# smpurkis/PyTorch-Face-Detection-from-Scratch

Measured on AMD Instinct MI355X. Metric: train imgs/sec (PoolResnet 480^2, bs=256 per GPU), higher is better.
Workload: dtype f32 (3x3 convs: bf16x3 split MFMA, fp32 accumulate)

## Files before the change

### include/fdet.h

```cpp
#ifndef FDET_H
#define FDET_H

#include <stddef.h>
#include <stdint.h>

#ifdef __cplusplus
extern "C" {
#endif

#define FDET_VERSION 100
#define FDET_OK 0
#define FDET_EINVAL (-1)
#define FDET_ELAUNCH (-2)
#define FDET_EWORKSPACE (-3)

int fdet_version(void);
const char* fdet_last_error(void);


int fdet_encode_targets(const float* boxes, const int32_t* box_offset, int B, int S,
                        float img_w, float img_h, float* out, void* stream);

int fdet_yolo_loss_fwd_bwd(const float* pred, const float* gt, int B, int S,
                           float* loss_per_image, float* loss_sum, float* grad_pred,
                           float grad_scale, void* stream);

int fdet_decode(const float* maps, int B, int S, float prob_threshold, float img_w, float img_h,
                float* scores, float* boxes, int32_t* counts, void* stream);

int fdet_nms(const float* boxes, const float* scores, const int32_t* counts, int B, int Kmax,
             double iou_threshold, int32_t* keep, int32_t* keep_counts, void* stream);

int fdet_reduce_bounding_boxes(const float* maps, int B, int S, float prob_threshold,
                               double iou_threshold, float img_w, float img_h,
                               float* out, int32_t* out_counts, void* stream);

int fdet_step_metrics(const float* gt, const int32_t* gt_counts, const float* pred,
                      const int32_t* pred_counts, int B, int Kmax, float* per_image,
                      float* totals, void* stream);

int fdet_u8_to_f32_norm(const uint8_t* in, float* out, size_t n, void* stream);


int fdet_adam_step(float* param, const float* grad, float* exp_avg, float* exp_avg_sq, size_t n,
                   int step, double lr, double beta1, double beta2, double eps, float grad_scale,
                   void* stream);

int fdet_ssd_num_priors(const int* h_patch_sizes, int nscales);
int fdet_ssd_encode_targets(const float* boxes, const int32_t* box_offsets, int B, const int* h_patch_sizes,
                            int nscales, float img_w, float img_h, float* out, void* stream);
size_t fdet_ssd_loss_ws_bytes(int B);
int fdet_ssd_loss_fwd_bwd(const float* pred, const float* target, int B, int P, int neg_pos_ratio, float* loss,
                          float* grad, uint8_t* mask, void* ws, size_t ws_bytes, void* stream);
int fdet_ssd_loss_parts(const float* pred, const float* target, int B, int P, int neg_pos_ratio, float* grad, uint8_t* mask,
                        double* sums, void* ws, size_t ws_bytes, void* stream);
int fdet_ssd_loss_finish(const double* sums, float* loss, float* grad, size_t n_grad, void* ws, size_t ws_bytes, void* stream);
int fdet_ssd_reduce_bounding_boxes(const float* x, int B, const int* h_patch_sizes, int nscales, int with_priors,
                                   float prob_threshold, double iou_threshold, float img_w, float img_h,
                                   float* out, int32_t* out_counts, void* stream);
int fdet_ssd_reduce_bounding_boxes_priors(const float* x, int B, const int* h_patch_sizes, int nscales, int with_priors,
                                          const float* priors, float prob_threshold, double iou_threshold, float img_w,
                                          float img_h, float* out, int32_t* out_counts, void* stream);

int fdet_ssd_head_pack_fwd(const float* z, int N, int CP, int ps, int prior_start, int P, float* y, void* stream);
int fdet_ssd_head_pack_bwd(const float* dy, const float* y, int N, int CP, int ps, int prior_start, int P, float* dz,
                           void* stream);

int fdet_resize_bilinear_u8_norm(const uint8_t* src, float* dst, int N, int C, int Hs, int Ws,
                                 int Hd, int Wd, void* stream);
int fdet_resize_bilinear_f32_norm(const float* src, float* dst, int N, int C, int Hs, int Ws,
                                  int Hd, int Wd, float divisor, void* stream);


int fdet_pack_conv3x3_weights(const float* w, int Cout, int Cin, float* wpk_fwd, float* wpk_bwd,
                              void* stream);

int fdet_conv3x3_fwd(const float* x, const float* wpk, const float* bias, float* y_full,
                     const float* skip, const float* drop_scale, float* y_out,
                     int N, int Cin, int Cout, int H, int W, int pool, float slope, void* stream);

int fdet_conv3x3_dgrad(const float* dz, const float* wpk, const float* act, const float* add,
                       float* dx, int N, int Cin, int Cout, int H, int W, float slope, void* stream);

int fdet_pack_conv3x3_weights_bf16x3(const float* w, int Cout, int Cin, void* wpk_fwd, void* wpk_bwd,
                                     void* stream);
int fdet_pack_conv3x3_weights_bf16x3_batched(const float* const* h_w, int L, int Cout, int Cin,
                                             void* const* h_wpk_fwd, void* const* h_wpk_bwd, void* stream);
int fdet_conv3x3_fwd_bf16x3(const float* x, const void* wpk, const float* bias, float* y_full,
                            const float* skip, const float* drop_scale, float* y_out,
                            int N, int Cin, int Cout, int H, int W, int pool, float slope, void* stream);
int fdet_conv3x3_dgrad_bf16x3(const float* dz, const void* wpk, const float* act, const float* add,
                              float* dx, int N, int Cin, int Cout, int H, int W, float slope, void* stream);

size_t fdet_conv3x3_wgrad_ws_bytes(int N, int Cin, int Cout, int H, int W);
int fdet_conv3x3_wgrad(const float* x, const float* dz, float* dW, float* db, void* ws,
                       size_t ws_bytes, int N, int Cin, int Cout, int H, int W, void* stream);

size_t fdet_conv3x3_wgrad_bf16x3_ws_bytes(int N, int Cin, int Cout, int H, int W);
int fdet_conv3x3_wgrad_bf16x3(const float* x, const float* dz, float* dW, float* db, void* ws,
                              size_t ws_bytes, int N, int Cin, int Cout, int H, int W, void* stream);

size_t fdet_conv3x3_wgrad_bf16x3_batched_ws_bytes(int L, int N, int Cin, int Cout, int H, int W);
int fdet_conv3x3_wgrad_bf16x3_plan(int N, int Cin, int Cout, int H, int W, int L, int* out, int n);
int fdet_conv3x3_wgrad_bf16x3_batched(const float* const* h_x, const float* const* h_dz, float* const* h_dW,
                                      float* const* h_db, int L, void* ws, size_t ws_bytes,
                                      int N, int Cin, int Cout, int H, int W, void* stream);

int fdet_block_chain_supported(int F, int H, int W);
int fdet_block_chain_ok(int N, int F, int H, int W, int ps);
int fdet_block_chain_fwd_bf16x3(const float* x, const void* const* h_wpk1, const float* const* h_b1,
                                const void* const* h_wpk2, const float* const* h_b2,
                                const float* const* h_scale, float* const* h_a, float* const* h_c,
                                float* const* h_out, int nblocks, int N, int F, int H, int W, float slope,
                                void* stream);
int fdet_block_chain_bwd_bf16x3(const float* dout, const void* const* h_wpk1b, const void* const* h_wpk2b,
                                const float* const* h_scale, const float* const* h_a, const float* const* h_c,
                                float* const* h_dz1, float* const* h_dz2, float* dx, int nblocks, int N, int F,
                                int H, int W, float slope, void* stream);

int fdet_block_chain_fwd_ps(const void* x, int x_is_ps, const void* const* h_wpk1, const float* const* h_b1,
                            const void* const* h_wpk2, const float* const* h_b2, const float* const* h_scale,
                            void* const* h_a_ps, void* const* h_c_ps, void* const* h_out_ps, float* out_last,
                            int nblocks, int N, int F, int H, int W, float slope, void* stream);
int fdet_block_chain_bwd_ps(const float* dout, const void* const* h_wpk1b, const void* const* h_wpk2b,
                            const float* const* h_scale, const void* const* h_a_ps, const void* const* h_c_ps,
                            void* const* h_dz1_ps, void* const* h_dz2_ps, float* dx, int nblocks, int N, int F,
                            int H, int W, float slope, void* stream);

int fdet_block_tail_fwd(const float* c, const float* x, const float* drop_scale, float* out,
                        int N, int F, int H, int W, int pool, void* stream);

int fdet_conv3x3_pool_fusion_ok(int N, int Cin, int Cout, int H, int W);
int fdet_conv3x3_x3_last_route(int* out, int n);
int fdet_conv3x3_ps_ok(int N, int Cin, int Cout, int H, int W, int pooled);
int fdet_conv3x3_fwd_pool_bf16x3(const float* x, const void* wpk, const float* bias, const float* skip,
                                 const float* drop_scale, float* out_pooled, unsigned char* route, int N, int Cin,
                                 int Cout, int H, int W, float slope, void* stream);
int fdet_conv3x3_dgrad_unpool_bf16x3(const float* dz, const void* wpk, const float* dout_pooled,
                                     const unsigned char* route, float* dx, int N, int Cin, int Cout, int H, int W,
                                     float slope, void* stream);
int fdet_pool_route_bwd(const float* dout_pooled, const unsigned char* route, const float* drop_scale, float* dz2,
                        int N, int F, int H, int W, float slope, void* stream);

size_t fdet_ps_bytes(int N, int C, int H, int W);
size_t fdet_ps_image0_offset(int N, int C, int H, int W);
int fdet_ps_from_f32(const float* x, void* ps, int N, int C, int H, int W, void* stream);
int fdet_ps_to_f32(const void* ps, float* x, int N, int C, int H, int W, void* stream);
int fdet_ps_strips(int W);
int fdet_ps_halo_exchange(void* ps, int N, int C, int H, int W, int zero_only, int hi_only, void* stream);
int fdet_conv3x3_ps_fwd(const void* x_ps, const void* wpk, const float* bias, void* y_ps, int N, int Cin, int Cout,
                        int H, int W, float slope, void* stream);
int fdet_conv3x3_ps_dgrad_act(const void* dz_ps, const void* wpk, const void* act_ps, void* dx_ps, int N, int Cin,
                              int Cout, int H, int W, float slope, void* stream);

int fdet_conv3x3_ps_fwd_pool(const void* x_ps, const void* wpk, const float* bias, const void* skip_ps,
                             const float* drop_scale, void* pool_ps, float* pool_f32, unsigned char* route8, int N, int Cin,
                             int Cout, int H, int W, float slope, void* stream);
int fdet_pool_route_bwd_ps(const float* dout_pooled, const unsigned char* route8, const float* drop_scale, void* dz2_ps,
                           int N, int C, int H, int W, float slope, void* stream);
int fdet_conv3x3_ps_dgrad_unpool(const void* dz_ps, const void* wpk, const float* dout_pooled, const unsigned char* route8,
                                 float* dx, int N, int Cin, int Cout, int H, int W, float slope, void* stream);
int fdet_stem_fwd_ps(const float* x, const float* w, const float* bias, void* y_ps, int N, int Cin, int F, int H, int W,
                     int k, int stride, int pad, void* stream);
size_t fdet_conv3x3_wgrad_ps_ws_bytes(int L, int N, int C, int H, int W);
int fdet_conv3x3_wgrad_ps_batched(const void* const* h_x, const void* const* h_dz, float* const* h_dW, float* const* h_db,
                                  int L, int N, int C, int H, int W, void* ws, size_t ws_bytes, void* stream);

size_t fdet_pointwise_packed_bytes(int Cout, int Cin);
int fdet_pack_pointwise_weights_bf16x3(const float* w, int Cout, int Cin, void* wpk_fwd, void* wpk_bwd, void* stream);
int fdet_pointwise_fwd_bf16x3(const float* x, const void* wpk_fwd, const float* bias, float* y, int N, int Cin, int Cout,
                              int P, float slope, void* stream);
int fdet_pointwise_dgrad_bf16x3(const float* dz, const void* wpk_bwd, const float* add, float* dx, int N, int Cin,
                                int Cout, int P, void* stream);
size_t fdet_pointwise_wgrad_ws_bytes(int N, int Cin, int Cout, int P);
int fdet_pointwise_wgrad_bf16x3(const float* x, const float* dz, float* dW, float* db, void* ws, size_t ws_bytes, int N,
                                int Cin, int Cout, int P, void* stream);
int fdet_pointwise_fwd_bf16(const float* x, const void* wpk_fwd, const float* bias, float* y, int N, int Cin, int Cout,
                            int P, float slope, void* stream);
int fdet_pointwise_dgrad_bf16(const float* dz, const void* wpk_bwd, const float* add, float* dx, int N, int Cin,
                              int Cout, int P, void* stream);
int fdet_pointwise_wgrad_bf16(const float* x, const float* dz, float* dW, float* db, void* ws, size_t ws_bytes, int N,
                              int Cin, int Cout, int P, void* stream);

int fdet_mb_stem(const void* x, int x_is_u8, const float* w, const float* bias, void* y, int N, int H, int W, void* stream);
int fdet_mb_depthwise(const void* x, const float* w, const float* bias, void* y, float* pool, int N, int H, int W, int C,
                      int K, int stride, int act, void* stream);
int fdet_mb_depthwise_pool_slots(int N, int H, int W, int C, int K, int stride);
int fdet_mb_se_gate(const float* pool, int slots, int HW, const float* w1, const float* b1, const float* w2, const float* b2,
                    int N, int C, int R, float* gate, void* stream);
int fdet_mb_pointwise(const void* x, const void* w, const float* bias, const float* gate, const void* res, void* y, int N,
                      int P, int Cin, int Cout, int act, void* stream);
size_t fdet_mb_head_ws_bytes(int N, int S);
int fdet_mb_head(const void* f, const void* w, const float* bias, float* y, void* ws, size_t ws_bytes, int N, int S, int C,
                 void* stream);

int fdet_block_tail_bwd(const float* dout, const float* c, const float* x, const float* drop_scale,
                        float* dz2, float* de, int N, int F, int H, int W, int pool, float slope,
                        void* stream);

size_t fdet_stem_ws_bytes(int N, int Cin, int F, int H, int W, int k, int stride, int pad);
int fdet_stem_fwd(const float* x, const float* w, const float* bias, float* y, void* ws, size_t ws_bytes,
                  int N, int Cin, int F, int H, int W, int k, int stride, int pad, void* stream);
int fdet_stem_fwd_bf16x3(const float* x, const float* w, const float* bias, float* y, void* ws, size_t ws_bytes,
                         int N, int Cin, int F, int H, int W, int k, int stride, int pad, void* stream);
int fdet_stem_wgrad(const float* x, const float* dy, float* dW, float* db, void* ws, size_t ws_bytes,
                    int N, int Cin, int F, int H, int W, int k, int stride, int pad, void* stream);
int fdet_stem_wgrad_bf16x3(const float* x, const float* dy, float* dW, float* db, void* ws, size_t ws_bytes,
                           int N, int Cin, int F, int H, int W, int k, int stride, int pad, void* stream);

int fdet_head_fwd(const float* x, const float* drop_scale, const float* w, const float* bias,
                  float* y, int N, int F, int H, int W, int k, int pad, void* stream);
size_t fdet_head_bwd_ws_bytes(int N, int F, int H, int W, int k, int pad);
int fdet_head_bwd(const float* x, const float* drop_scale, const float* w, const float* y,
                  const float* dy, float* dx, float* dW, float* db, void* ws, size_t ws_bytes,
                  int N, int F, int H, int W, int k, int pad, void* stream);

int fdet_conv3x3_ps_fwd_p16(const void* x_ps, const void* wpk, const float* bias, void* y_ps, int N, int Cin,
                            int Cout, int H, int W, float slope, void* stream);
int fdet_conv3x3_ps_dgrad_act_p16(const void* dz_ps, const void* wpk, const void* act_ps, void* dx_ps, int N,
                                  int Cin, int Cout, int H, int W, float slope, void* stream);
int fdet_conv3x3_ps_fwd_pool_p16(const void* x_ps, const void* wpk, const float* bias, const void* skip_ps,
                                 const float* drop_scale, void* pool_ps, float* pool_f32, unsigned char* route8,
                                 int N, int Cin, int Cout, int H, int W, float slope, void* stream);
int fdet_conv3x3_ps_dgrad_unpool_p16(const void* dz_ps, const void* wpk, const float* dout_pooled,
                                     const unsigned char* route8, float* dx, int N, int Cin, int Cout, int H, int W,
                                     float slope, void* stream);
int fdet_pool_route_bwd_ps_p16(const float* dout_pooled, const unsigned char* route8, const float* drop_scale,
                               void* dz2_ps, int N, int C, int H, int W, float slope, void* stream);
int fdet_stem_fwd_ps_p16(const float* x, const float* w, const float* bias, void* y_ps, int N, int Cin, int F, int H,
                         int W, int k, int stride, int pad, void* stream);
int fdet_stem_fwd_ps_u8(const unsigned char* frames, const float* w, const float* bias, void* y_ps, int N, int Cin, int F, int H,
                        int W, int k, int stride, int pad, int precision16, void* stream);
int fdet_stem_wgrad_bf16(const float* x, const float* dy, float* dW, float* db, void* ws, size_t ws_bytes,
                         int N, int Cin, int F, int H, int W, int k, int stride, int pad, void* stream);
int fdet_stem_fwd_ps_ok(int N, int Cin, int F, int H, int W, int k, int stride, int pad, int precision16, int u8);
int fdet_stem_wgrad_x3_ok(int N, int Cin, int F, int H, int W, int k, int stride, int pad, int precision16);
#define FDET_STEM_VALU_K10 1
#define FDET_STEM_VALU_K3_GENERIC 2
#define FDET_STEM_VALU_K3_SCALAR 3
#define FDET_STEM_MFMA 4
#define FDET_STEM_X3_SINGLE 5
#define FDET_STEM_X3_PIPE 6
#define FDET_STEM_K3_MATRIX 7
#define FDET_STEM_K3_PS_FWD 8
int fdet_stem_last_route(int* out, int n);
int fdet_conv3x3_wgrad_ps_batched_p16(const void* const* h_x, const void* const* h_dz, float* const* h_dW,
                                      float* const* h_db, int L, int N, int C, int H, int W, void* ws,
                                      size_t ws_bytes, void* stream);
int fdet_block_chain_fwd_ps_p16(const void* x, int x_is_ps, const void* const* h_wpk1, const float* const* h_b1,
                                const void* const* h_wpk2, const float* const* h_b2, const float* const* h_scale,
                                void* const* h_a_ps, void* const* h_c_ps, void* const* h_out_ps, float* out_last,
                                int nblocks, int N, int F, int H, int W, float slope, void* stream);
int fdet_block_chain_bwd_ps_p16(const float* dout, const void* const* h_wpk1b, const void* const* h_wpk2b,
                                const float* const* h_scale, const void* const* h_a_ps, const void* const* h_c_ps,
                                void* const* h_dz1_ps, void* const* h_dz2_ps, float* dx, int nblocks, int N, int F,
                                int H, int W, float slope, void* stream);

int fdet_conv3x3_fwd_bf16(const float* x, const void* wpk, const float* bias, float* y_full,
                          const float* skip, const float* drop_scale, float* y_out, int N, int Cin,
                          int Cout, int H, int W, int pool, float slope, void* stream);
int fdet_conv3x3_dgrad_bf16(const float* dz, const void* wpk, const float* act, const float* add,
                            float* dx, int N, int Cin, int Cout, int H, int W, float slope, void* stream);
int fdet_conv3x3_fwd_pool_bf16(const float* x, const void* wpk, const float* bias, const float* skip,
                               const float* drop_scale, float* out_pooled, unsigned char* route, int N,
                               int Cin, int Cout, int H, int W, float slope, void* stream);
int fdet_conv3x3_dgrad_unpool_bf16(const float* dz, const void* wpk, const float* dout_pooled,
                                   const unsigned char* route, float* dx, int N, int Cin, int Cout,
                                   int H, int W, float slope, void* stream);
int fdet_conv3x3_wgrad_bf16(const float* x, const float* dz, float* dW, float* db, void* ws,
                            size_t ws_bytes, int N, int Cin, int Cout, int H, int W, void* stream);
int fdet_conv3x3_wgrad_bf16_batched(const float* const* h_x, const float* const* h_dz, float* const* h_dW,
                                    float* const* h_db, int L, void* ws, size_t ws_bytes, int N, int Cin,
                                    int Cout, int H, int W, void* stream);

int fdet_mbt_stem_fwd(const float* x, const float* w, float* z, int N, int H, int W, void* stream);
size_t fdet_mbt_taps_ws_bytes(int C, int k);
int fdet_mbt_stem_wgrad(const float* x, const float* dz, float* dW, void* ws, size_t ws_bytes, int N, int H, int W, void* stream);
int fdet_mbt_dw_fwd(const float* x, const float* w, float* z, int N, int C, int H, int W, int k, int s, void* stream);
int fdet_mbt_dw_bwd(const float* x, const float* dz, const float* w, float* dx, float* dW, void* ws, size_t ws_bytes, int N,
                    int C, int H, int W, int k, int s, void* stream);
size_t fdet_mbt_bn_ws_bytes(int C);
int fdet_mbt_bn_fwd(const float* z, const float* gamma, const float* beta, float* running_mean, float* running_var,
                    float momentum, float eps, float* save_mean, float* save_invstd, const float* residual, float* y,
                    void* ws, size_t ws_bytes, int N, int C, int P, int act, void* stream);
int fdet_mbt_bn_bwd(const float* z, const float* dy, const float* gamma, const float* beta, const float* save_mean,
                    const float* save_invstd, float* dz, float* dgamma, float* dbeta, void* ws, size_t ws_bytes, int N,
                    int C, int P, int act, void* stream);
int fdet_mbt_se_fwd(const float* x, const float* w1, const float* b1, const float* w2, const float* b2, float* pooled,
                    float* hidden, float* pre, float* y, int N, int C, int R, int P, void* stream);
int fdet_mbt_se_bwd(const float* x, const float* dy, const float* pooled, const float* hidden, const float* pre,
                    const float* w1, const float* w2, float* dx, float* dw1, float* db1, float* dw2, float* db2, void* ws,
                    size_t ws_bytes, int N, int C, int R, int P, void* stream);

int fdet_head_loss_fused_supported(int F, int H, int W, int k, int pad);
size_t fdet_head_loss_fused_ws_bytes(int N, int F, int H, int W, int k, int pad);
int fdet_head_loss_fused(const float* x, const float* drop_scale, const float* w, const float* bias,
                         const float* gt, float* y, float* loss_per_image, float* loss_sum, float* dx,
                         float* dW, float* db, void* ws, size_t ws_bytes, int N, int F, int H, int W, int k,
                         int pad, void* stream);

int fdet_dropout_scales(float* out, size_t n, float p, uint64_t seed, uint64_t offset, void* stream);

int fdet_dropout_scales_layers(float* out, int n, int nlayers, const int* channels, const float* p,
                               uint64_t seed, uint64_t base, uint64_t first_image, void* stream);

typedef struct fdet_aug_image {
  int64_t offset;
  int32_t h, w;
} fdet_aug_image;

#define FDET_AUG_FLIP 1
#define FDET_AUG_ROTATE 2
#define FDET_AUG_BRIGHTNESS 4
#define FDET_AUG_NOISE 8
#define FDET_AUG_GLASS 16
#define FDET_AUG_MOTION 32
#define FDET_AUG_CROP 64
#define FDET_AUG_CROP_FALLBACK 128

typedef struct fdet_aug_params {
  int32_t image;
  int32_t flags;
  int32_t crop_x0, crop_y0, crop_w, crop_h;
  float angle, cos_a, sin_a;
  float alpha, beta;
  float sigma;
  uint32_t key;
  int32_t motion_k;
  float motion_w[49];
  int32_t reserved;
} fdet_aug_params;

int fdet_aug_warp(const uint8_t* bank, const fdet_aug_image* table, const fdet_aug_image* h_table, int n_images,
                  const fdet_aug_params* params, const fdet_aug_params* h_params, int B, int Ho, int Wo,
                  uint32_t seed, uint8_t* mid, void* stream);
int fdet_aug_finish(const uint8_t* mid, const fdet_aug_params* params, const fdet_aug_params* h_params, int B, int Ho,
                    int Wo, uint32_t seed, uint8_t* out_u8, float* out_f32, void* stream);
int fdet_aug_boxes(const float* boxes, const int32_t* box_offset, const fdet_aug_image* table,
                   const fdet_aug_image* h_table, int n_images, const fdet_aug_params* params,
                   const fdet_aug_params* h_params, int B, int Ho, int Wo, int max_rows, float* rows,
                   int32_t* out_offset, void* stream);

#define FDET_EVAL_MAX_THRESHOLDS 10
#define FDET_EVAL_MAX_DET 4864
#define FDET_EVAL_MAX_GT 4096
#define FDET_EVAL_MAX_BINS 4096
#define FDET_EVAL_N_GT 0
#define FDET_EVAL_N_IMAGES 1
#define FDET_EVAL_N_DET 2
#define FDET_EVAL_N_REJECTED 3
#define FDET_EVAL_N_COUNTERS 4
int fdet_eval_match(const float* pred, const int32_t* pred_counts, int B, int Kmax, const float* gt_rows,
                    const int32_t* gt_offset, int gt_cap, int max_gt, const float* iou_thresholds, int T,
                    int n_bins, uint32_t* tp, uint32_t* fp, uint64_t* counters, int32_t* match, void* stream);

#define FDET_EVAL_WIDER_MAX_SUBSETS 8
#define FDET_EVAL_WIDER_N_IMAGES 0
#define FDET_EVAL_WIDER_N_DET 1
#define FDET_EVAL_WIDER_N_REJECTED 2
#define FDET_EVAL_WIDER_N_COUNTERS 3
int fdet_eval_wider(const float* pred, const int32_t* pred_counts, int B, int Kmax, const float* pred_scale,
                    const float* gt_rows, const int32_t* gt_offset, int gt_cap, const uint32_t* gt_subsets,
                    int n_subsets, int max_gt, double iou_threshold, const double* score_norm, int n_bins,
                    uint32_t* proposals, uint32_t* hits, uint64_t* counters, void* stream);

typedef struct fdet_tile {
  int32_t image, x0, y0, w, h;
} fdet_tile;

int fdet_tile_gather(const uint8_t* bank, const fdet_aug_image* table, const fdet_aug_image* h_table, int n_images,
                     const fdet_tile* tiles, const fdet_tile* h_tiles, int T, int Ho, int Wo, uint8_t* frames,
                     void* stream);

#define FDET_TILE_MAX_CANDIDATES 4864
int fdet_tile_merge(const float* rows, const int32_t* counts, const fdet_tile* tiles, const int32_t* tile_offset,
                    int n_images, int T, int K, int Ho, int Wo, const fdet_aug_image* table, float edge_margin,
                    double iou_threshold, int Kout, float* out, int32_t* out_counts, uint64_t* rejected, void* stream);

int fdet_tile_gather_flags(const uint8_t* bank, const fdet_aug_image* table, const fdet_aug_image* h_table, int n_images,
                           const fdet_tile* tiles, const fdet_tile* h_tiles, const uint8_t* flags, const uint8_t* h_flags,
                           int T, int Ho, int Wo, uint8_t* frames, void* stream);

int fdet_tile_merge_vote(const float* rows, const int32_t* counts, const fdet_tile* tiles, const uint8_t* flags,
                         const int32_t* tile_offset, int n_images, int T, int K, int Ho, int Wo,
                         const fdet_aug_image* table, float edge_margin, double iou_threshold, int min_votes, int vote,
                         int Kout, float* out, int32_t* out_votes, int32_t* out_counts, uint64_t* rejected, void* stream);

int fdet_render_boxes(const uint8_t* src, const fdet_aug_image* src_table, const fdet_aug_image* h_src_table,
                      const float* rows, const int32_t* counts, const int32_t* h_counts, int n_images, int K, uint8_t* dst,
                      const fdet_aug_image* dst_table, const fdet_aug_image* h_dst_table, int outline, int pixelate,
                      int blocks, int red, int green, int blue, int32_t* ws, void* stream);

#define FDET_TRACK_SLOTS     128
#define FDET_TRACK_MAX_DETS  256
#define FDET_TRACK_MAX_COORD 16384

typedef struct fdet_track {
  int32_t id, x1q, y1q, x2q, y2q, hits, misses, born;
  float score;
  int32_t reserved[3];
} fdet_track;
typedef struct fdet_track_seq {
  int32_t next_id, frame, dropped, reserved;
} fdet_track_seq;

size_t fdet_track_state_bytes(int n_seq);

int fdet_track_update(const float* rows, const int32_t* counts, const int32_t* seq_offset, const int32_t* h_seq_offset,
                      int n_seq, int T, int K, double iou_threshold, int alpha256, int max_misses, int min_hits,
                      int emit_misses, float birth_score, void* state, float* out_rows, int32_t* out_ids,
                      int32_t* out_misses, int32_t* out_counts, int32_t* det_ids, uint64_t* rejected, void* stream);

#define FDET_CHIP_MIN_SIZE 8
#define FDET_CHIP_MAX_SIZE 256
#define FDET_CHIP_MAX_SIDE 8192
#define FDET_CHIP_MAX_CHIPS (1 << 20)

typedef struct fdet_chip_info {
  int32_t image, row;
  int32_t wx0, wy0, S;
  int32_t inside256;
  int32_t flags;
  int32_t reserved;
  int64_t sharp;
} fdet_chip_info;

int fdet_chip_extract(const uint8_t* bank, const fdet_aug_image* table, const fdet_aug_image* h_table, int n_images,
                      const float* rows, const int32_t* counts, const int32_t* h_counts,
                      const int32_t* chip_offset, const int32_t* h_chip_offset, int K, int C, int margin256,
                      int planar, uint8_t* chips, fdet_chip_info* info, void* stream);

typedef struct fdet_chip_best {
  int32_t id;
  int32_t frame, image_wx0, image_wy0, S, inside256, seen, reserved;
  int64_t sharp;
} fdet_chip_best;

size_t fdet_chip_gallery_bytes(int n_seq, int G);

int fdet_chip_best_update(const uint8_t* chips, const fdet_chip_info* info, int M, int C, const int32_t* ids, int K,
                          const int32_t* seq_offset, const int32_t* h_seq_offset, int n_seq, const int32_t* frame_base,
                          int G, int min_side, int min_inside256, void* gallery, uint8_t* gallery_chips,
                          uint64_t* scratch, uint64_t* overflow, void* stream);

int fdet_sepblock_plan(int F, int H, int W, int pool, int* out, int n);
int fdet_sepblock_fwd(const float* x, const void* w1_pk, const float* wd, const void* w2_pk, const float* drop_scale,
                      float* out, float* a_save, float* b_save, unsigned char* route, int N, int F, int H, int W,
                      int pool, float slope, void* stream);
int fdet_sepblock_gate_bwd(const float* g, const float* act, const float* drop_scale, float* out, int N, int F, int P,
                           float slope, void* stream);
int fdet_sepblock_lrelu(const float* z, float* y, size_t n, float slope, void* stream);

#define FDET_JPEG_UNSUPPORTED (-4)
#define FDET_JPEG_ECORRUPT (-5)

typedef struct fdet_jpeg_info_t {
  int32_t width, height, ncomp;
  int32_t restart_interval;
  int32_t hs[3], vs[3];
  int32_t blocks_w[3], blocks_h[3];
  int32_t mcus_x, mcus_y;
  int64_t coef_count;
  uint16_t qt[3][64];
} fdet_jpeg_info_t;

int fdet_jpeg_info(const uint8_t* bytes, size_t n, fdet_jpeg_info_t* out);

int fdet_jpeg_entropy_decode(const uint8_t* bytes, size_t n, int16_t* coef, size_t capacity);

typedef struct fdet_jpeg_desc {
  int64_t bank_offset;
  int64_t coef_offset[3];
  int64_t plane_offset[3];
  int32_t width, height, ncomp;
  int32_t hs, vs;
  int32_t blocks_w[3], blocks_h[3];
  int32_t reserved;
  uint16_t qt[3][64];
} fdet_jpeg_desc;

int fdet_jpeg_reconstruct(const int16_t* coef, size_t coef_count, const fdet_jpeg_desc* descs, const fdet_jpeg_desc* h_descs,
                          int n_images, uint8_t* workspace, size_t workspace_bytes, uint8_t* bank, size_t bank_bytes,
                          void* stream);

#ifdef __cplusplus
}
#endif
#endif
```

### pytorch-face-detection-from-scratch_amd/_native.py

```python
from __future__ import annotations

import ctypes
import os
import re
import subprocess
from typing import Optional

import torch

_HERE = os.path.dirname(os.path.abspath(__file__))
LIB_PATH = os.environ.get("FDET_LIB_PATH") or os.path.join(_HERE, "lib", "libfdet_hip.so")
HEADER_PATH = os.path.join(os.path.dirname(_HERE), "include", "fdet.h")


class FdetError(RuntimeError):
    pass


def build(verbose: bool = False) -> str:
    cmd = ["make", "-C", os.path.join(_HERE, "csrc"), "-j", str(min(8, os.cpu_count() or 1))]
    r = subprocess.run(cmd, capture_output=True, text=True)
    if verbose or r.returncode != 0:
        print(r.stdout[-4000:])
        print(r.stderr[-8000:])
    if r.returncode != 0:
        raise FdetError("building libfdet_hip.so failed (see compiler output above)")
    return LIB_PATH


_c = ctypes
_P, _I, _F, _D, _SZ, _U64, _U32 = _c.c_void_p, _c.c_int, _c.c_float, _c.c_double, _c.c_size_t, _c.c_uint64, _c.c_uint32

SIGNATURES = {
    "fdet_version": (_I, []),
    "fdet_last_error": (_c.c_char_p, []),
    "fdet_encode_targets": (_I, [_P, _P, _I, _I, _F, _F, _P, _P]),
    "fdet_yolo_loss_fwd_bwd": (_I, [_P, _P, _I, _I, _P, _P, _P, _F, _P]),
    "fdet_decode": (_I, [_P, _I, _I, _F, _F, _F, _P, _P, _P, _P]),
    "fdet_nms": (_I, [_P, _P, _P, _I, _I, _D, _P, _P, _P]),
    "fdet_reduce_bounding_boxes": (_I, [_P, _I, _I, _F, _D, _F, _F, _P, _P, _P]),
    "fdet_step_metrics": (_I, [_P, _P, _P, _P, _I, _I, _P, _P, _P]),
    "fdet_ssd_num_priors": (_I, [_P, _I]),
    "fdet_ssd_encode_targets": (_I, [_P, _P, _I, _P, _I, _F, _F, _P, _P]),
    "fdet_ssd_loss_ws_bytes": (_SZ, [_I]),
    "fdet_ssd_loss_fwd_bwd": (_I, [_P, _P, _I, _I, _I, _P, _P, _P, _P, _SZ, _P]),
    "fdet_ssd_loss_parts": (_I, [_P, _P, _I, _I, _I, _P, _P, _P, _P, _SZ, _P]),
    "fdet_ssd_loss_finish": (_I, [_P, _P, _P, _SZ, _P, _SZ, _P]),
    "fdet_ssd_reduce_bounding_boxes": (_I, [_P, _I, _P, _I, _I, _F, _D, _F, _F, _P, _P, _P]),
    "fdet_ssd_reduce_bounding_boxes_priors": (_I, [_P, _I, _P, _I, _I, _P, _F, _D, _F, _F, _P, _P, _P]),
    "fdet_ssd_head_pack_fwd": (_I, [_P, _I, _I, _I, _I, _I, _P, _P]),
    "fdet_ssd_head_pack_bwd": (_I, [_P, _P, _I, _I, _I, _I, _I, _P, _P]),
    "fdet_u8_to_f32_norm": (_I, [_P, _P, _SZ, _P]),
    "fdet_resize_bilinear_u8_norm": (_I, [_P, _P, _I, _I, _I, _I, _I, _I, _P]),
    "fdet_resize_bilinear_f32_norm": (_I, [_P, _P, _I, _I, _I, _I, _I, _I, _F, _P]),
    "fdet_adam_step": (_I, [_P, _P, _P, _P, _SZ, _I, _D, _D, _D, _D, _F, _P]),
    "fdet_pack_conv3x3_weights": (_I, [_P, _I, _I, _P, _P, _P]),
    "fdet_conv3x3_fwd": (_I, [_P, _P, _P, _P, _P, _P, _P, _I, _I, _I, _I, _I, _I, _F, _P]),
    "fdet_conv3x3_dgrad": (_I, [_P, _P, _P, _P, _P, _I, _I, _I, _I, _I, _F, _P]),
    "fdet_pack_conv3x3_weights_bf16x3": (_I, [_P, _I, _I, _P, _P, _P]),
    "fdet_pack_conv3x3_weights_bf16x3_batched": (_I, [_P, _I, _I, _I, _P, _P, _P]),
    "fdet_conv3x3_fwd_bf16x3": (_I, [_P, _P, _P, _P, _P, _P, _P, _I, _I, _I, _I, _I, _I, _F, _P]),
    "fdet_conv3x3_dgrad_bf16x3": (_I, [_P, _P, _P, _P, _P, _I, _I, _I, _I, _I, _F, _P]),
    "fdet_conv3x3_fwd_pool_bf16x3": (_I, [_P, _P, _P, _P, _P, _P, _P, _I, _I, _I, _I, _I, _F, _P]),
    "fdet_conv3x3_dgrad_unpool_bf16x3": (_I, [_P, _P, _P, _P, _P, _I, _I, _I, _I, _I, _F, _P]),
    "fdet_pool_route_bwd": (_I, [_P, _P, _P, _P, _I, _I, _I, _I, _F, _P]),
    "fdet_conv3x3_pool_fusion_ok": (_I, [_I, _I, _I, _I, _I]),
    "fdet_conv3x3_x3_last_route": (_I, [_P, _I]),
    "fdet_conv3x3_ps_ok": (_I, [_I, _I, _I, _I, _I, _I]),
    "fdet_stem_fwd_ps_ok": (_I, [_I, _I, _I, _I, _I, _I, _I, _I, _I, _I]),
    "fdet_stem_last_route": (_I, [_P, _I]),
    "fdet_stem_wgrad_x3_ok": (_I, [_I, _I, _I, _I, _I, _I, _I, _I, _I]),
    "fdet_ps_bytes": (_SZ, [_I, _I, _I, _I]),
    "fdet_ps_image0_offset": (_SZ, [_I, _I, _I, _I]),
    "fdet_ps_from_f32": (_I, [_P, _P, _I, _I, _I, _I, _P]),
    "fdet_ps_to_f32": (_I, [_P, _P, _I, _I, _I, _I, _P]),
    "fdet_ps_strips": (_I, [_I]),
    "fdet_ps_halo_exchange": (_I, [_P, _I, _I, _I, _I, _I, _I, _P]),
    "fdet_conv3x3_ps_fwd": (_I, [_P, _P, _P, _P, _I, _I, _I, _I, _I, _F, _P]),
    "fdet_conv3x3_ps_dgrad_act": (_I, [_P, _P, _P, _P, _I, _I, _I, _I, _I, _F, _P]),
    "fdet_conv3x3_ps_fwd_pool": (_I, [_P, _P, _P, _P, _P, _P, _P, _P, _I, _I, _I, _I, _I, _F, _P]),
    "fdet_pool_route_bwd_ps": (_I, [_P, _P, _P, _P, _I, _I, _I, _I, _F, _P]),
    "fdet_conv3x3_ps_dgrad_unpool": (_I, [_P, _P, _P, _P, _P, _I, _I, _I, _I, _I, _F, _P]),
    "fdet_stem_fwd_ps": (_I, [_P, _P, _P, _P, _I, _I, _I, _I, _I, _I, _I, _I, _P]),
    "fdet_conv3x3_wgrad_ps_ws_bytes": (_SZ, [_I, _I, _I, _I, _I]),
    "fdet_conv3x3_wgrad_ps_batched": (_I, [_P, _P, _P, _P, _I, _I, _I, _I, _I, _P, _SZ, _P]),
    "fdet_pointwise_packed_bytes": (_SZ, [_I, _I]),
    "fdet_pack_pointwise_weights_bf16x3": (_I, [_P, _I, _I, _P, _P, _P]),
    "fdet_pointwise_fwd_bf16x3": (_I, [_P, _P, _P, _P, _I, _I, _I, _I, _F, _P]),
    "fdet_pointwise_dgrad_bf16x3": (_I, [_P, _P, _P, _P, _I, _I, _I, _I, _P]),
    "fdet_pointwise_wgrad_ws_bytes": (_SZ, [_I, _I, _I, _I]),
    "fdet_pointwise_wgrad_bf16x3": (_I, [_P, _P, _P, _P, _P, _SZ, _I, _I, _I, _I, _P]),
    "fdet_pointwise_fwd_bf16": (_I, [_P, _P, _P, _P, _I, _I, _I, _I, _F, _P]),
    "fdet_pointwise_dgrad_bf16": (_I, [_P, _P, _P, _P, _I, _I, _I, _I, _P]),
    "fdet_pointwise_wgrad_bf16": (_I, [_P, _P, _P, _P, _P, _SZ, _I, _I, _I, _I, _P]),
    "fdet_mb_stem": (_I, [_P, _I, _P, _P, _P, _I, _I, _I, _P]),
    "fdet_mb_depthwise": (_I, [_P, _P, _P, _P, _P, _I, _I, _I, _I, _I, _I, _I, _P]),
    "fdet_mb_depthwise_pool_slots": (_I, [_I, _I, _I, _I, _I, _I]),
    "fdet_mb_se_gate": (_I, [_P, _I, _I, _P, _P, _P, _P, _I, _I, _I, _P, _P]),
    "fdet_mb_pointwise": (_I, [_P, _P, _P, _P, _P, _P, _I, _I, _I, _I, _I, _P]),
    "fdet_mb_head_ws_bytes": (_SZ, [_I, _I]),
    "fdet_mb_head": (_I, [_P, _P, _P, _P, _P, _SZ, _I, _I, _I, _P]),
    "fdet_conv3x3_wgrad_ws_bytes": (_SZ, [_I, _I, _I, _I, _I]),
    "fdet_conv3x3_wgrad": (_I, [_P, _P, _P, _P, _P, _SZ, _I, _I, _I, _I, _I, _P]),
    "fdet_conv3x3_wgrad_bf16x3_ws_bytes": (_SZ, [_I, _I, _I, _I, _I]),
    "fdet_conv3x3_wgrad_bf16x3": (_I, [_P, _P, _P, _P, _P, _SZ, _I, _I, _I, _I, _I, _P]),
    "fdet_conv3x3_wgrad_bf16x3_batched_ws_bytes": (_SZ, [_I, _I, _I, _I, _I, _I]),
    "fdet_conv3x3_wgrad_bf16x3_plan": (_I, [_I, _I, _I, _I, _I, _I, _P, _I]),
    "fdet_conv3x3_wgrad_bf16x3_batched": (_I, [_P, _P, _P, _P, _I, _P, _SZ, _I, _I, _I, _I, _I, _P]),
    "fdet_block_chain_supported": (_I, [_I, _I, _I]),
    "fdet_block_chain_ok": (_I, [_I, _I, _I, _I, _I]),
    "fdet_block_chain_fwd_bf16x3": (_I, [_P, _P, _P, _P, _P, _P, _P, _P, _P, _I, _I, _I, _I, _I, _F, _P]),
    "fdet_block_chain_bwd_bf16x3": (_I, [_P, _P, _P, _P, _P, _P, _P, _P, _P, _I, _I, _I, _I, _I, _F, _P]),
    "fdet_block_chain_fwd_ps": (_I, [_P, _I, _P, _P, _P, _P, _P, _P, _P, _P, _P, _I, _I, _I, _I, _I, _F, _P]),
    "fdet_block_chain_bwd_ps": (_I, [_P, _P, _P, _P, _P, _P, _P, _P, _P, _I, _I, _I, _I, _I, _F, _P]),
    "fdet_block_tail_fwd": (_I, [_P, _P, _P, _P, _I, _I, _I, _I, _I, _P]),
    "fdet_block_tail_bwd": (_I, [_P, _P, _P, _P, _P, _P, _I, _I, _I, _I, _I, _F, _P]),
    "fdet_stem_ws_bytes": (_SZ, [_I, _I, _I, _I, _I, _I, _I, _I]),
    "fdet_stem_fwd": (_I, [_P, _P, _P, _P, _P, _SZ, _I, _I, _I, _I, _I, _I, _I, _I, _P]),
    "fdet_stem_fwd_bf16x3": (_I, [_P, _P, _P, _P, _P, _SZ, _I, _I, _I, _I, _I, _I, _I, _I, _P]),
    "fdet_stem_wgrad": (_I, [_P, _P, _P, _P, _P, _SZ, _I, _I, _I, _I, _I, _I, _I, _I, _P]),
    "fdet_stem_wgrad_bf16x3": (_I, [_P, _P, _P, _P, _P, _SZ, _I, _I, _I, _I, _I, _I, _I, _I, _P]),
    "fdet_head_fwd": (_I, [_P, _P, _P, _P, _P, _I, _I, _I, _I, _I, _I, _P]),
    "fdet_head_bwd_ws_bytes": (_SZ, [_I, _I, _I, _I, _I, _I]),
    "fdet_head_bwd": (_I, [_P, _P, _P, _P, _P, _P, _P, _P, _P, _SZ, _I, _I, _I, _I, _I, _I, _P]),
    "fdet_conv3x3_ps_fwd_p16": (_I, [_P, _P, _P, _P, _I, _I, _I, _I, _I, _F, _P]),
    "fdet_conv3x3_ps_dgrad_act_p16": (_I, [_P, _P, _P, _P, _I, _I, _I, _I, _I, _F, _P]),
    "fdet_conv3x3_ps_fwd_pool_p16": (_I, [_P, _P, _P, _P, _P, _P, _P, _P, _I, _I, _I, _I, _I, _F, _P]),
    "fdet_conv3x3_ps_dgrad_unpool_p16": (_I, [_P, _P, _P, _P, _P, _I, _I, _I, _I, _I, _F, _P]),
    "fdet_pool_route_bwd_ps_p16": (_I, [_P, _P, _P, _P, _I, _I, _I, _I, _F, _P]),
    "fdet_stem_fwd_ps_p16": (_I, [_P, _P, _P, _P, _I, _I, _I, _I, _I, _I, _I, _I, _P]),
    "fdet_stem_fwd_ps_u8": (_I, [_P, _P, _P, _P, _I, _I, _I, _I, _I, _I, _I, _I, _I, _P]),
    "fdet_stem_wgrad_bf16": (_I, [_P, _P, _P, _P, _P, _SZ, _I, _I, _I, _I, _I, _I, _I, _I, _P]),
    "fdet_conv3x3_wgrad_ps_batched_p16": (_I, [_P, _P, _P, _P, _I, _I, _I, _I, _I, _P, _SZ, _P]),
    "fdet_block_chain_fwd_ps_p16": (_I, [_P, _I, _P, _P, _P, _P, _P, _P, _P, _P, _P, _I, _I, _I, _I, _I, _F, _P]),
    "fdet_block_chain_bwd_ps_p16": (_I, [_P, _P, _P, _P, _P, _P, _P, _P, _P, _I, _I, _I, _I, _I, _F, _P]),
    "fdet_conv3x3_fwd_bf16": (_I, [_P, _P, _P, _P, _P, _P, _P, _I, _I, _I, _I, _I, _I, _F, _P]),
    "fdet_conv3x3_dgrad_bf16": (_I, [_P, _P, _P, _P, _P, _I, _I, _I, _I, _I, _F, _P]),
    "fdet_conv3x3_fwd_pool_bf16": (_I, [_P, _P, _P, _P, _P, _P, _P, _I, _I, _I, _I, _I, _F, _P]),
    "fdet_conv3x3_dgrad_unpool_bf16": (_I, [_P, _P, _P, _P, _P, _I, _I, _I, _I, _I, _F, _P]),
    "fdet_conv3x3_wgrad_bf16": (_I, [_P, _P, _P, _P, _P, _SZ, _I, _I, _I, _I, _I, _P]),
    "fdet_conv3x3_wgrad_bf16_batched": (_I, [_P, _P, _P, _P, _I, _P, _SZ, _I, _I, _I, _I, _I, _P]),
    "fdet_mbt_stem_fwd": (_I, [_P, _P, _P, _I, _I, _I, _P]),
    "fdet_mbt_taps_ws_bytes": (_SZ, [_I, _I]),
    "fdet_mbt_stem_wgrad": (_I, [_P, _P, _P, _P, _SZ, _I, _I, _I, _P]),
    "fdet_mbt_dw_fwd": (_I, [_P, _P, _P, _I, _I, _I, _I, _I, _I, _P]),
    "fdet_mbt_dw_bwd": (_I, [_P, _P, _P, _P, _P, _P, _SZ, _I, _I, _I, _I, _I, _I, _P]),
    "fdet_mbt_bn_ws_bytes": (_SZ, [_I]),
    "fdet_mbt_bn_fwd": (_I, [_P, _P, _P, _P, _P, _F, _F, _P, _P, _P, _P, _P, _SZ, _I, _I, _I, _I, _P]),
    "fdet_mbt_bn_bwd": (_I, [_P, _P, _P, _P, _P, _P, _P, _P, _P, _P, _SZ, _I, _I, _I, _I, _P]),
    "fdet_mbt_se_fwd": (_I, [_P, _P, _P, _P, _P, _P, _P, _P, _P, _I, _I, _I, _I, _P]),
    "fdet_mbt_se_bwd": (_I, [_P, _P, _P, _P, _P, _P, _P, _P, _P, _P, _P, _P, _P, _SZ, _I, _I, _I, _I, _P]),
    "fdet_head_loss_fused_supported": (_I, [_I, _I, _I, _I, _I]),
    "fdet_head_loss_fused_ws_bytes": (_SZ, [_I, _I, _I, _I, _I, _I]),
    "fdet_head_loss_fused": (_I, [_P, _P, _P, _P, _P, _P, _P, _P, _P, _P, _P, _P, _SZ, _I, _I, _I, _I, _I, _I, _P]),
    "fdet_dropout_scales": (_I, [_P, _SZ, _F, _U64, _U64, _P]),
    "fdet_dropout_scales_layers": (_I, [_P, _I, _I, _P, _P, _U64, _U64, _U64, _P]),
    "fdet_aug_warp": (_I, [_P, _P, _P, _I, _P, _P, _I, _I, _I, _U32, _P, _P]),
    "fdet_aug_finish": (_I, [_P, _P, _P, _I, _I, _I, _U32, _P, _P, _P]),
    "fdet_aug_boxes": (_I, [_P, _P, _P, _P, _I, _P, _P, _I, _I, _I, _I, _P, _P, _P]),
    "fdet_eval_match": (_I, [_P, _P, _I, _I, _P, _P, _I, _I, _P, _I, _I, _P, _P, _P, _P, _P]),
    "fdet_eval_wider": (_I, [_P, _P, _I, _I, _P, _P, _P, _I, _P, _I, _I, _D, _P, _I, _P, _P, _P, _P]),
    "fdet_tile_gather": (_I, [_P, _P, _P, _I, _P, _P, _I, _I, _I, _P, _P]),
    "fdet_tile_merge": (_I, [_P, _P, _P, _P, _I, _I, _I, _I, _I, _P, _F, _D, _I, _P, _P, _P, _P]),
    "fdet_tile_gather_flags": (_I, [_P, _P, _P, _I, _P, _P, _P, _P, _I, _I, _I, _P, _P]),
    "fdet_tile_merge_vote": (_I, [_P, _P, _P, _P, _P, _I, _I, _I, _I, _I, _P, _F, _D, _I, _I, _I, _P, _P, _P, _P, _P]),
    "fdet_render_boxes": (_I, [_P, _P, _P, _P, _P, _P, _I, _I, _P, _P, _P, _I, _I, _I, _I, _I, _I, _P, _P]),
    "fdet_track_state_bytes": (_SZ, [_I]),
    "fdet_track_update": (_I, [_P, _P, _P, _P, _I, _I, _I, _D, _I, _I, _I, _I, _F, _P, _P, _P, _P, _P, _P, _P, _P]),
    "fdet_chip_extract": (_I, [_P, _P, _P, _I, _P, _P, _P, _P, _P, _I, _I, _I, _I, _P, _P, _P]),
    "fdet_chip_gallery_bytes": (_SZ, [_I, _I]),
    "fdet_chip_best_update": (_I, [_P, _P, _I, _I, _P, _I, _P, _P, _I, _P, _I, _I, _I, _P, _P, _P, _P, _P]),
    "fdet_sepblock_plan": (_I, [_I, _I, _I, _I, _P, _I]),
    "fdet_sepblock_fwd": (_I, [_P, _P, _P, _P, _P, _P, _P, _P, _P, _I, _I, _I, _I, _I, _F, _P]),
    "fdet_sepblock_gate_bwd": (_I, [_P, _P, _P, _P, _I, _I, _I, _F, _P]),
    "fdet_sepblock_lrelu": (_I, [_P, _P, _SZ, _F, _P]),
    "fdet_jpeg_info": (_I, [_P, _SZ, _P]),
    "fdet_jpeg_entropy_decode": (_I, [_P, _SZ, _P, _SZ]),
    "fdet_jpeg_reconstruct": (_I, [_P, _SZ, _P, _P, _I, _P, _SZ, _P, _SZ, _P]),
}


def header_symbols() -> list:
    txt = open(HEADER_PATH).read()
    txt = re.sub(r"/\*.*?\*/", "", txt, flags=re.S)
    return sorted(set(re.findall(r"\b(fdet_[a-z0-9_]+)\s*\(", txt)))


_lib: Optional[ctypes.CDLL] = None


def lib() -> ctypes.CDLL:
    global _lib
    if _lib is None:
        if not os.path.exists(LIB_PATH):
            raise FdetError(f"{LIB_PATH} is missing: run `python -c 'import __graft_entry__ as g; g.build()'` "
                            "(hipcc --offload-arch=gfx950).  There is no CPU fallback.")
        L = ctypes.CDLL(LIB_PATH)
        for name, (res, args) in SIGNATURES.items():
            fn = getattr(L, name)
            fn.restype = res
            fn.argtypes = args
        if L.fdet_version() != 100:
            raise FdetError(f"libfdet_hip.so version {L.fdet_version()} != 100")
        _lib = L
    return _lib


def hip_runtimes_mapped() -> list:
    out = set()
    with open("/proc/self/maps") as f:
        for line in f:
            if "libamdhip64" in line:
                out.add(line.split()[-1])
    return sorted(out)


def check(rc: int, what: str = "") -> None:
    if rc != 0:
        msg = lib().fdet_last_error().decode(errors="replace")
        raise FdetError(f"{what} failed with code {rc}: {msg}")


def ptr(t: Optional[torch.Tensor], dtype=torch.float32) -> Optional[int]:
    if t is None:
        return None
    if not isinstance(t, torch.Tensor):
        raise TypeError(f"expected a torch.Tensor, got {type(t)}")
    if not t.is_cuda:
        raise FdetError("libfdet_hip.so works on GPU memory only; got a CPU tensor (no CPU fallback exists)")
    if t.dtype != dtype:
        raise TypeError(f"expected dtype {dtype}, got {t.dtype}")
    if not t.is_contiguous():
        raise TypeError("expected a contiguous tensor")
    return t.data_ptr()


def stream() -> int:
    return torch.cuda.current_stream().cuda_stream
```

### pytorch-face-detection-from-scratch_amd/convstack.py

```python
from __future__ import annotations

from dataclasses import dataclass
from typing import Dict, List, Optional

import torch

from . import hotpath as hp
from . import ps as psm

F32 = torch.float32


@dataclass
class StackGeometry:
    kind: str
    filters: int
    in_ch: int
    H: int
    W: int
    S: int
    num_blocks: int
    stem_k: int
    stem_s: int
    stem_p: int
    head_k: int
    head_p: int
    pool_mult: int
    strict_grid: bool = True

    def levels(self):
        h0 = (self.H + 2 * self.stem_p - self.stem_k) // self.stem_s + 1
        w0 = (self.W + 2 * self.stem_p - self.stem_k) // self.stem_s + 1
        if h0 != w0:
            raise ValueError("square inputs only (reference swaps width/height, datasets/utils.py:107)")
        out, h = [], h0
        for _ in range(self.num_blocks):
            pool = 2 if h > self.pool_mult * self.S else 1
            if pool == 2 and h % 2:
                raise ValueError(f"cannot 2x2-pool an odd {h}x{h} map")
            out.append((h, pool))
            h //= pool
        s_out = h + 2 * self.head_p - self.head_k + 1
        if s_out != self.S and self.strict_grid:
            raise ValueError(f"input {self.H}x{self.W} with this stem/head reaches a {s_out}x{s_out} grid, "
                             f"not num_of_patches={self.S}")
        if s_out <= 0:
            raise ValueError(f"input {self.H}x{self.W} with this stem/head leaves no output grid")
        return h0, out


PARAM_ORDER_DOC = "conv1.{weight,bias}, residual_blocks.k.conv{1,2}.{weight,bias}, out.{weight,bias}"


class KernelTimer:

    def __init__(self):
        self.rec = {}

    def span(self, name, flops=0.0, nbytes=0.0):
        return _Span(self, name, flops, nbytes)

    def summary(self):
        torch.cuda.synchronize()
        out = {}
        for name, (evs, flops, nbytes) in self.rec.items():
            out[name] = (len(evs), sum(a.elapsed_time(b) for a, b in evs), flops / len(evs), nbytes / len(evs))
        return out


class _Span:
    def __init__(self, timer, name, flops, nbytes):
        self.t, self.name, self.flops, self.nbytes = timer, name, flops, nbytes

    def __enter__(self):
        self.a = torch.cuda.Event(enable_timing=True)
        self.b = torch.cuda.Event(enable_timing=True)
        self.a.record()

    def __exit__(self, *exc):
        self.b.record()
        rec = self.t.rec.setdefault(self.name, [[], 0.0, 0.0])
        rec[0].append((self.a, self.b))
        rec[1] += self.flops
        rec[2] += self.nbytes


class _NoSpan:
    def __enter__(self):
        return None

    def __exit__(self, *exc):
        return False


_NOSPAN = _NoSpan()


class _PsScope(list):

    def __init__(self, pool):
        super().__init__()
        self.pool = pool

    def release(self):
        for key, t in self:
            self.pool.setdefault(key, []).append(t)
        self.clear()

    def __del__(self):
        self.release()


class ConvStack:

    def __init__(self, geo: StackGeometry):
        self.geo = geo
        self.h0, self.lv = geo.levels()
        self._packed_key = None
        self._wpk: Dict[str, torch.Tensor] = {}
        self._ws: Dict[str, torch.Tensor] = {}
        self.slope = 0.2
        self.timer: Optional[KernelTimer] = None
        import os
        want = os.environ.get("FDET_PRECISION", "bf16x3")
        self.x3 = (want in ("bf16x3", "bf16")) and hp.x3_supported(geo.filters, geo.filters)
        self.pool_fusion = self.x3 and os.environ.get("FDET_POOL_FUSION", "1") != "0"
        self.ps = self.pool_fusion and geo.filters == 64 and os.environ.get("FDET_PS", "1") != "0"
        self._ps_pool: Dict[tuple, list] = {}
        self.ps_strips = self.ps and os.environ.get("FDET_PS_STRIPS", "1") != "0"
        self.p16 = self.x3 and want == "bf16"
        self._cur_N = 1
        self.head_fused = self.x3 and os.environ.get("FDET_HEAD_FUSED", "1") != "0"
        self._zero_ws: Dict[str, torch.Tensor] = {}

    def set_precision(self, name: str) -> None:
        if name not in ("bf16x3", "bf16"):
            raise ValueError("precision must be 'bf16x3' or 'bf16'")
        if name == "bf16" and not self.x3:
            raise ValueError("precision16 needs the bf16 matrix-core conv kernels: this engine runs the exact-fp32 path "
                             f"(FDET_PRECISION=f32, or {self.geo.filters} channels is not a multiple of 16)")
        self.p16 = name == "bf16"
        self._ps_pool.clear()

    def u8_frames_ok(self) -> bool:
        g = self.geo
        return bool(self.ps and self.x3 and self.lv and 30 <= self.h0 <= 62 and self.lv[0][1] == 2 and g.W % 4 == 0 and
                    hp.stem_x3_supported(g.in_ch, g.W, g.stem_k, g.stem_s, g.stem_p) and g.filters == 64)

    def head_loss_fusable(self) -> bool:
        g = self.geo
        hl = self.lv[-1][0] // self.lv[-1][1] if self.lv else self.h0
        return self.head_fused and hp.head_loss_fused_supported(g.filters, hl, hl, g.head_k, g.head_p)

    def _t(self, kind: str, N: int, h: int, flops: float = 0.0, nbytes: float = 0.0):
        if self.timer is None:
            return _NOSPAN
        return self.timer.span(f"{kind}@{h}x{h}", flops, nbytes)

    def _conv_flops(self, N: int, h: int) -> float:
        F_ = self.geo.filters
        return 2.0 * N * F_ * F_ * 9 * h * h

    def _act_bytes(self, N: int, h: int, tensors: float) -> float:
        return 4.0 * N * self.geo.filters * h * h * tensors

    def _ensure_packed(self, P: Dict[str, torch.Tensor], force: bool = False):
        key = (self.x3,) + tuple((P[k].data_ptr(), P[k]._version) for k in sorted(P) if k.endswith("weight"))
        if not force and key == self._packed_key:
            return
        F_ = self.geo.filters
        nf, nb = hp.packed_sizes(F_, F_)
        dev = P["conv1.weight"].device
        names = [f"residual_blocks.{k}.conv{j}" for k in range(self.geo.num_blocks) for j in (1, 2)]
        for name in names:
            if name + ".f" not in self._wpk:
                self._wpk[name + ".f"] = torch.empty(nf, dtype=F32, device=dev)
                self._wpk[name + ".b"] = torch.empty(nb, dtype=F32, device=dev)
        if self.x3:
            hp.pack_conv3x3_weights_batched([P[nm + ".weight"] for nm in names], [self._wpk[nm + ".f"] for nm in names],
                                            [self._wpk[nm + ".b"] for nm in names])
        else:
            for name in names:
                hp.pack_conv3x3_weights(P[name + ".weight"], self._wpk[name + ".f"], self._wpk[name + ".b"], x3=False)
        self._packed_key = key

    def mark_params_dirty(self):
        self._packed_key = None

    def _workspace(self, name: str, nbytes: int, dev) -> torch.Tensor:
        n = (nbytes + 3) // 4
        t = self._ws.get(name)
        if t is None or t.numel() < n or t.device != dev:
            t = torch.empty(max(n, 4), dtype=F32, device=dev)
            self._ws[name] = t
        return t

    def _fused_pool(self, hk: int, N: int = 1) -> bool:
        return self.pool_fusion and hp.pool_fusion_supported(self.geo.filters, self.geo.filters, hk, hk, N)

    def _ps_block(self, k: int) -> bool:
        if not self.ps or k >= len(self.lv):
            return False
        hk, pool = self.lv[k]
        if pool != 2 or hk % 2 or hk < 30:
            return False
        if self._cur_N * self.geo.filters * hk * hk * 4 >= 2 ** 31:
            return False
        if hk > 62:
            return self.ps_strips and psm.strips_of(hk)[0] > 1 and psm.conv3x3_wgrad_ps_ws_bytes(1, self._cur_N, self.geo.filters, hk, hk) > 0
        return self._fused_pool(hk, self._cur_N)

    def _stem_ps(self) -> bool:
        g = self.geo
        return self._ps_block(0) and self.x3 and \
            ((not self._strips(self.h0) and hp.stem_x3_supported(g.in_ch, g.W, g.stem_k, g.stem_s, g.stem_p)) or
             hp.stem_k3_fwd_ps_supported(g.in_ch, g.filters, g.H, g.W, g.stem_k, g.stem_s, g.stem_p))

    def _stem_wgrad_kind(self):
        g = self.geo
        x3 = self.x3 and ((g.W % 16 == 0 and hp.stem_x3_supported(g.in_ch, g.W, g.stem_k, g.stem_s, g.stem_p)) or
                          hp.stem_k3_wgrad_x3_supported(g.in_ch, g.filters, g.H, g.W, g.stem_k, g.stem_s, g.stem_p))
        return x3, self.p16 and x3 and 48 < self.h0 <= 60

    def _strips(self, hk: int) -> bool:
        return hk > 62

    def _ps_chain(self, k: int) -> bool:
        if not self.ps or k >= len(self.lv) or self._chain_run(k) <= 1:
            return False
        hk = self.lv[k][0]
        return psm.conv3x3_wgrad_ps_ws_bytes(1, self._cur_N, self.geo.filters, hk, hk) > 0 and \
            self._cur_N * self.geo.filters * hk * hk * 4 < 2 ** 31

    def _ps_take(self, scope: "_PsScope", N: int, C: int, H: int, W: int, dev) -> "psm.PsTensor":
        key = (N, C, H, W, str(dev))
        free = self._ps_pool.setdefault(key, [])
        t = free.pop() if free else psm.PsTensor(N, C, H, W, dev)
        scope.append((key, t))
        return t

    def _chain_run(self, k: int) -> int:
        import os
        if not self.x3 or os.environ.get("FDET_CHAIN", "1") == "0":
            return 0
        hk, pool = self.lv[k]
        if pool != 1 or not hp.block_chain_supported(self.geo.filters, hk, hk):
            return 0
        run = 1
        while k + run < len(self.lv) and self.lv[k + run] == (hk, 1) and run < 16:
            run += 1
        return run

    def forward(self, x: torch.Tensor, P: Dict[str, torch.Tensor], masks: Optional[Dict[str, torch.Tensor]] = None,
                save: bool = False, loss_targets: Optional[torch.Tensor] = None, G: Optional[Dict[str, torch.Tensor]] = None,
                u8_frames: bool = False):
        g = self.geo
        if x.dim() != 4 or tuple(x.shape[1:]) != (g.in_ch, g.H, g.W):
            raise ValueError(f"expected input (N,{g.in_ch},{g.H},{g.W}), got {tuple(x.shape)}")
        if u8_frames:
            if x.dtype != torch.uint8 or save or not self.u8_frames_ok():
                raise ValueError("u8_frames: uint8 input, inference only, PoolResnet stem on the pre-split path")
            x = x.contiguous()
        elif x.dtype != F32 or not x.is_contiguous():
            x = x.to(F32).contiguous()
        self._ensure_packed(P)
        N, F_, dev = x.shape[0], g.filters, x.device
        if N != self._cur_N:
            self._ps_pool.clear()
            self._cur_N = N
        ws = self._workspace("stem", hp.stem_ws_bytes(N, g.in_ch, F_, g.H, g.W, g.stem_k, g.stem_s, g.stem_p), dev)
        stem_ps = self._stem_ps()
        if u8_frames and not stem_ps:
            x = hp.u8_to_f32_norm(x)
        h = torch.empty(N, F_, self.h0, self.h0, dtype=F32, device=dev) if not stem_ps else None
        stem_flops = 2.0 * N * F_ * g.in_ch * g.stem_k * g.stem_k * self.h0 * self.h0
        stem_bytes = 4.0 * N * (g.in_ch * g.H * g.W + F_ * self.h0 * self.h0)
        scope = _PsScope(self._ps_pool)
        h_ps = None
        stem_x3 = self.x3 and hp.stem_x3_supported(g.in_ch, g.W, g.stem_k, g.stem_s, g.stem_p)
        with self._t("stem_fwd", N, self.h0, stem_flops, stem_bytes):
            if stem_ps:
                h, h_ps = None, self._ps_take(scope, N, F_, self.h0, self.h0, dev)
                psm.stem_fwd_ps(x, P["conv1.weight"], P["conv1.bias"], h_ps, g.stem_k, g.stem_s, g.stem_p, p16=self.p16)
            else:
                hp.stem_fwd(x, P["conv1.weight"], P["conv1.bias"], h, ws, g.stem_k, g.stem_s, g.stem_p, x3=stem_x3)
        saved = {"x": x, "blocks": [], "masks": masks, "ps_scope": scope, "p16": self.p16} if save else None
        k = -1
        while k + 1 < len(self.lv):
            k += 1
            hk, pool = self.lv[k]
            if self._ps_block(k):
                name = f"residual_blocks.{k}"
                sc = masks[name] if masks is not None else None
                if h_ps is None:
                    h_ps = psm.PsTensor.from_f32(h, out=self._ps_take(scope, N, F_, hk, hk, dev))
                a_ps = self._ps_take(scope, N, F_, hk, hk, dev)
                with self._t("conv3x3_fwd", N, hk, self._conv_flops(N, hk), self._act_bytes(N, hk, 2)):
                    psm.conv3x3_ps_fwd(h_ps, self._wpk[name + ".conv1.f"], P[name + ".conv1.bias"], a_ps, self.slope, p16=self.p16)
                    psm.halo_exchange(a_ps, p16=self.p16)
                nxt = (self._ps_block(k + 1) or self._ps_chain(k + 1)) and not self._strips(hk)
                out_ps = self._ps_take(scope, N, F_, hk // 2, hk // 2, dev) if nxt else None
                out = None if nxt else torch.empty(N, F_, hk // 2, hk // 2, dtype=F32, device=dev)
                route = psm.route8_like(N, F_, hk, hk, dev) if save else None
                with self._t("conv3x3_fwd_pool", N, hk, self._conv_flops(N, hk), self._act_bytes(N, hk, 2 + 0.25 + (1 / 16 if save else 0))):
                    psm.conv3x3_ps_fwd_pool(a_ps, self._wpk[name + ".conv2.f"], P[name + ".conv2.bias"], h_ps, sc, out_ps, out,
                                            route, self.slope, p16=self.p16)
                if save:
                    saved["blocks"].append((h_ps, a_ps, route))
                h, h_ps = out, out_ps
                continue
            run = self._chain_run(k)
            if run > 1 and self._ps_chain(k):
                names = [f"residual_blocks.{kk}" for kk in range(k, k + run)]
                if h_ps is None:
                    h_ps = psm.PsTensor.from_f32(h, out=self._ps_take(scope, N, F_, hk, hk, dev))
                a_l = [self._ps_take(scope, N, F_, hk, hk, dev) for _ in names] if save else None
                c_l = [self._ps_take(scope, N, F_, hk, hk, dev) for _ in names] if save else None
                o_l = [self._ps_take(scope, N, F_, hk, hk, dev) for _ in names[:-1]] if save else None
                out = torch.empty(N, F_, hk, hk, dtype=F32, device=dev)
                with self._t("chain_fwd", N, hk, 2 * run * self._conv_flops(N, hk), self._act_bytes(N, hk, 1 + (2.5 * run if save else 1))):
                    psm.block_chain_fwd_ps(h_ps, [self._wpk[nm + ".conv1.f"] for nm in names], [P[nm + ".conv1.bias"] for nm in names],
                                           [self._wpk[nm + ".conv2.f"] for nm in names], [P[nm + ".conv2.bias"] for nm in names],
                                           [masks[nm] for nm in names] if masks is not None else None, a_l, c_l, o_l, out, self.slope,
                                           p16=self.p16)
                if save:
                    for i in range(run):
                        saved["blocks"].append((h_ps if i == 0 else o_l[i - 1], a_l[i], c_l[i]))
                h, h_ps = out, None
                k += run - 1
                continue
            if run > 1:
                names = [f"residual_blocks.{kk}" for kk in range(k, k + run)]
                a_l = [torch.empty(N, F_, hk, hk, dtype=F32, device=dev) for _ in names] if save else None
                c_l = [torch.empty(N, F_, hk, hk, dtype=F32, device=dev) for _ in names] if save else None
                o_l = [torch.empty(N, F_, hk, hk, dtype=F32, device=dev) if (save or i == run - 1) else None
                       for i in range(run)]
                with self._t("chain_fwd", N, hk, 2 * run * self._conv_flops(N, hk), self._act_bytes(N, hk, 1 + (3 * run if save else 1))):
                    hp.block_chain_fwd(h, [self._wpk[nm + ".conv1.f"] for nm in names], [P[nm + ".conv1.bias"] for nm in names],
                                       [self._wpk[nm + ".conv2.f"] for nm in names], [P[nm + ".conv2.bias"] for nm in names],
                                       [masks[nm] for nm in names] if masks is not None else None, a_l, c_l, o_l, self.slope)
                if save:
                    for i in range(run):
                        saved["blocks"].append((h if i == 0 else o_l[i - 1], a_l[i], c_l[i]))
                h = o_l[-1]
                k += run - 1
                continue
            name = f"residual_blocks.{k}"
            sc = masks[name] if masks is not None else None
            a = torch.empty(N, F_, hk, hk, dtype=F32, device=dev)
            with self._t("conv3x3_fwd", N, hk, self._conv_flops(N, hk), self._act_bytes(N, hk, 2)):
                hp.conv3x3_fwd(h, self._wpk[name + ".conv1.f"], P[name + ".conv1.bias"], F_, y_full=a, slope=self.slope, x3=self.x3,
                               p16=self.p16)
            out = torch.empty(N, F_, hk // pool, hk // pool, dtype=F32, device=dev)
            if pool == 2 and self._fused_pool(hk, N):
                c = torch.empty(N, F_, hk // 2, hk // 2, dtype=torch.uint8, device=dev) if save else None
                with self._t("conv3x3_fwd_pool", N, hk, self._conv_flops(N, hk), self._act_bytes(N, hk, 2 + 0.25 + (1 / 16 if save else 0))):
                    hp.conv3x3_fwd_pool(a, self._wpk[name + ".conv2.f"], P[name + ".conv2.bias"], h, sc, out, c, self.slope,
                                        p16=self.p16)
            elif pool == 2:
                c = torch.empty_like(a)
                with self._t("conv3x3_fwd", N, hk, self._conv_flops(N, hk), self._act_bytes(N, hk, 2)):
                    hp.conv3x3_fwd(a, self._wpk[name + ".conv2.f"], P[name + ".conv2.bias"], F_, y_full=c, slope=self.slope, x3=self.x3,
                                   p16=self.p16)
                with self._t("tail_fwd", N, hk, 0.0, self._act_bytes(N, hk, 2.25)):
                    hp.block_tail_fwd(c, h, sc, out, 2)
            else:
                c = torch.empty_like(a) if save else None
                with self._t("conv3x3_fwd", N, hk, self._conv_flops(N, hk), self._act_bytes(N, hk, 4 if save else 3)):
                    hp.conv3x3_fwd(a, self._wpk[name + ".conv2.f"], P[name + ".conv2.bias"], F_, y_full=c, skip=h,
                                   drop_scale=sc, y_out=out, slope=self.slope, x3=self.x3, p16=self.p16)
            if save:
                saved["blocks"].append((h, a, c))
            h = out
        y = torch.empty(N, 5, g.S, g.S, dtype=F32, device=dev)
        if loss_targets is not None and save and G is not None and self.head_loss_fusable():
            if tuple(loss_targets.shape) != tuple(y.shape):
                raise ValueError(f"loss targets {tuple(loss_targets.shape)} != head output {tuple(y.shape)}")
            tg = loss_targets if (loss_targets.dtype == F32 and loss_targets.is_contiguous()) else loss_targets.to(F32).contiguous()
            hl = h.shape[2]
            nb = hp.head_loss_fused_ws_bytes(N, F_, hl, hl, g.head_k, g.head_p)
            ws = self._zero_ws.get("head_fused")
            if ws is None or ws.numel() * 4 != ((nb + 3) // 4) * 4 or ws.device != dev:
                ws = self._zero_ws["head_fused"] = torch.zeros((nb + 3) // 4, dtype=F32, device=dev)
            lpi = torch.empty(N, dtype=F32, device=dev)
            lsum = torch.empty(1, dtype=F32, device=dev)
            dout = torch.empty_like(h)
            macs = N * F_ * g.head_k ** 2 * (2 * 5 * g.S ** 2 + 5 * hl * hl)
            with self._t("head_loss_fused", N, hl, 2.0 * macs, self._act_bytes(N, hl, 2)):
                hp.head_loss_fused(h, masks["head"] if masks is not None else None, P["out.weight"], P["out.bias"], tg, y, lpi, lsum,
                                   dout, G["out.weight"], G["out.bias"], ws, g.head_k, g.head_p)
            saved["loss"] = (lpi, lsum)
            saved["head_dout"] = dout
        else:
            with self._t("head_fwd", N, h.shape[2], 2.0 * N * 5 * F_ * g.head_k ** 2 * g.S ** 2, self._act_bytes(N, h.shape[2], 1)):
                hp.head_fwd(h, masks["head"] if masks is not None else None, P["out.weight"], P["out.bias"], y, g.head_k, g.head_p)
        if save:
            saved["h_last"] = h
            saved["y"] = y
        else:
            scope.release()
        return y, saved

    def backward(self, saved, dy: torch.Tensor, P: Dict[str, torch.Tensor], G: Dict[str, torch.Tensor],
                 after_block=None) -> None:
        p16 = bool(saved.get("p16", self.p16))
        if p16 and not self.x3:
            raise ValueError("backward: the saved pass ran in precision16, which this engine cannot run")
        keep = self.p16
        self.p16 = p16
        try:
            self._backward(saved, dy, P, G, after_block)
        finally:
            self.p16 = keep

    def _backward(self, saved, dy, P, G, after_block) -> None:
        g = self.geo
        F_ = g.filters
        x, masks = saved["x"], saved["masks"]
        N, dev = x.shape[0], x.device
        self._cur_N = N
        h_last, y = saved["h_last"], saved["y"]
        if saved.get("head_dout") is not None:
            dout = saved["head_dout"]
        else:
            if dy is None or tuple(dy.shape) != tuple(y.shape):
                raise ValueError(f"dy shape {None if dy is None else tuple(dy.shape)} != y shape {tuple(y.shape)}")
            dy = dy.to(F32).contiguous()
            hl = h_last.shape[2]
            ws = self._workspace("head", hp.head_bwd_ws_bytes(N, F_, hl, hl, g.head_k, g.head_p), dev)
            dout = torch.empty_like(h_last)
            with self._t("head_bwd", N, hl, 4.0 * N * 5 * F_ * g.head_k ** 2 * g.S ** 2, self._act_bytes(N, hl, 2)):
                hp.head_bwd(h_last, masks["head"] if masks is not None else None, P["out.weight"], y, dy, dout,
                            G["out.weight"], G["out.bias"], ws, g.head_k, g.head_p)
        pending = []

        def flush(hk_):
            if not pending:
                return
            fl_ = self._conv_flops(N, hk_)
            for i0 in range(0, len(pending), 16):
                grp = pending[i0:i0 + 16]
                wsb_ = self._workspace("wgrad_batched", hp.conv3x3_wgrad_batched_ws_bytes(len(grp), N, F_, F_, hk_, hk_), dev)
                with self._t("conv3x3_wgrad", N, hk_, fl_ * len(grp), self._act_bytes(N, hk_, 2) * len(grp)):
                    hp.conv3x3_wgrad_batched([p_[0] for p_ in grp], [p_[1] for p_ in grp],
                                             [G[p_[2] + ".weight"] for p_ in grp], [G[p_[2] + ".bias"] for p_ in grp], wsb_,
                                             p16=self.p16)
            pending.clear()

        pending_ps = []

        def flush_ps(hk_):
            if not pending_ps:
                return
            fl_ = self._conv_flops(N, hk_)
            for i0 in range(0, len(pending_ps), 16):
                grp = pending_ps[i0:i0 + 16]
                wsb_ = self._workspace("wgrad_ps", psm.conv3x3_wgrad_ps_ws_bytes(len(grp), N, F_, hk_, hk_), dev)
                with self._t("conv3x3_wgrad", N, hk_, fl_ * len(grp), self._act_bytes(N, hk_, 2) * len(grp)):
                    psm.conv3x3_wgrad_ps_batched([p_[0] for p_ in grp], [p_[1] for p_ in grp],
                                                 [G[p_[2] + ".weight"] for p_ in grp], [G[p_[2] + ".bias"] for p_ in grp], wsb_,
                                                 p16=self.p16)
            pending_ps.clear()

        chain_start = {}
        kk = 0
        while kk < g.num_blocks:
            run = self._chain_run(kk)
            if run > 1:
                chain_start[kk + run - 1] = kk
                kk += run
            else:
                kk += 1
        k = g.num_blocks
        while k > 0:
            k -= 1
            hk, pool = self.lv[k]
            if k in chain_start and self._ps_chain(chain_start[k]):
                k0 = chain_start[k]
                ks = list(range(k0, k + 1))
                names = [f"residual_blocks.{q}" for q in ks]
                scope = saved.get("ps_scope")
                if scope is None:
                    scope = saved["ps_scope"] = _PsScope(self._ps_pool)

                def as_ps(t):
                    if isinstance(t, psm.PsTensor):
                        return t
                    return psm.PsTensor.from_f32(t.to(F32).contiguous(), out=self._ps_take(scope, N, F_, hk, hk, dev))
                x_l = [as_ps(saved["blocks"][q][0]) for q in ks]
                a_l = [as_ps(saved["blocks"][q][1]) for q in ks]
                c_l = [as_ps(saved["blocks"][q][2]) for q in ks]
                dz1_l = [self._ps_take(scope, N, F_, hk, hk, dev) for _ in ks]
                dz2_l = [self._ps_take(scope, N, F_, hk, hk, dev) for _ in ks]
                dx = torch.empty_like(dout)
                with self._t("chain_bwd", N, hk, 2 * len(ks) * self._conv_flops(N, hk), self._act_bytes(N, hk, 2 + 3 * len(ks))):
                    psm.block_chain_bwd_ps(dout, [self._wpk[nm + ".conv1.b"] for nm in names], [self._wpk[nm + ".conv2.b"] for nm in names],
                                           [masks[nm] for nm in names] if masks is not None else None, a_l, c_l, dz1_l, dz2_l, dx, self.slope,
                                           p16=self.p16)
                for i in reversed(range(len(ks))):
                    pending_ps.append((a_l[i], dz2_l[i], names[i] + ".conv2"))
                    pending_ps.append((x_l[i], dz1_l[i], names[i] + ".conv1"))
                dout = dx
                k = k0
                if k == 0 or self.lv[k - 1][0] != hk:
                    flush_ps(hk)
                    if after_block is not None:
                        for q in range(k, g.num_blocks):
                            if self.lv[q][0] == hk:
                                after_block(q)
                continue
            if k in chain_start:
                k0 = chain_start[k]
                ks = list(range(k0, k + 1))
                names = [f"residual_blocks.{q}" for q in ks]
                dz1_l = [torch.empty_like(saved["blocks"][q][1]) for q in ks]
                dz2_l = [torch.empty_like(saved["blocks"][q][1]) for q in ks]
                dx = torch.empty_like(dout)
                with self._t("chain_bwd", N, hk, 2 * len(ks) * self._conv_flops(N, hk), self._act_bytes(N, hk, 2 + 4 * len(ks))):
                    hp.block_chain_bwd(dout, [self._wpk[nm + ".conv1.b"] for nm in names], [self._wpk[nm + ".conv2.b"] for nm in names],
                                       [masks[nm] for nm in names] if masks is not None else None,
                                       [saved["blocks"][q][1] for q in ks], [saved["blocks"][q][2] for q in ks],
                                       dz1_l, dz2_l, dx, self.slope)
                for i in reversed(range(len(ks))):
                    q = ks[i]
                    pending.append((saved["blocks"][q][1], dz2_l[i], names[i] + ".conv2"))
                    pending.append((saved["blocks"][q][0], dz1_l[i], names[i] + ".conv1"))
                dout = dx
                k = k0
                if k == 0 or self.lv[k - 1][0] != hk:
                    flush(hk)
                    if after_block is not None:
                        for q in range(k, g.num_blocks):
                            if self.lv[q][0] == hk:
                                after_block(q)
                continue
            name = f"residual_blocks.{k}"
            xin, a, c = saved["blocks"][k]
            sc = masks[name] if masks is not None else None
            if self._ps_block(k) and c is not None and c.dtype == torch.uint8 and \
                    (isinstance(a, psm.PsTensor) or isinstance(xin, psm.PsTensor) or c.dim() == 5):
                scope = saved.get("ps_scope")
                if scope is None:
                    scope = saved["ps_scope"] = _PsScope(self._ps_pool)
                if not isinstance(xin, psm.PsTensor):
                    xin = psm.PsTensor.from_f32(xin.to(F32).contiguous(), out=self._ps_take(scope, N, F_, hk, hk, dev))
                if not isinstance(a, psm.PsTensor):
                    a = psm.PsTensor.from_f32(a.to(F32).contiguous(), out=self._ps_take(scope, N, F_, hk, hk, dev))
                strips = self._strips(hk)
                if c.dim() == 4:
                    if strips:
                        raise ValueError("routing bytes of a strip level are per strip (ps.route8_shape)")
                    c = c.view(N, F_ // 8, 8, hk // 2, hk // 2).permute(0, 1, 3, 4, 2).contiguous()
                fl = self._conv_flops(N, hk)

                def wgrad_now(x_, dz_, nm_, clean=False):
                    if not clean:
                        psm.halo_exchange(dz_, zero_only=True, p16=self.p16)
                    pending_ps.append((x_, dz_, nm_))
                    flush_ps(hk)
                    psm.halo_exchange(dz_, p16=self.p16)
                dz2 = self._ps_take(scope, N, F_, hk, hk, dev)
                with self._t("pool_route_bwd", N, hk, 0.0, self._act_bytes(N, hk, 1 + 0.25 + 1 / 16)):
                    psm.pool_route_bwd_ps(dout, c, sc, dz2, self.slope, p16=self.p16)
                if strips:
                    wgrad_now(a, dz2, name + ".conv2", clean=True)
                dz1 = self._ps_take(scope, N, F_, hk, hk, dev)
                with self._t("conv3x3_dgrad", N, hk, fl, self._act_bytes(N, hk, 3)):
                    psm.conv3x3_ps_dgrad_act(dz2, self._wpk[name + ".conv2.b"], a, dz1, self.slope, p16=self.p16)
                if strips:
                    wgrad_now(xin, dz1, name + ".conv1")
                dx = torch.empty(N, F_, hk, hk, dtype=F32, device=dev)
                with self._t("conv3x3_dgrad_unpool", N, hk, fl, self._act_bytes(N, hk, 2 + 0.25 + 1 / 16)):
                    psm.conv3x3_ps_dgrad_unpool(dz1, self._wpk[name + ".conv1.b"], dout, c, dx, self.slope, p16=self.p16)
                if not strips:
                    pending_ps.append((a, dz2, name + ".conv2"))
                    pending_ps.append((xin, dz1, name + ".conv1"))
                dout = dx
                if k == 0 or self.lv[k - 1][0] != hk or not self._ps_block(k - 1):
                    flush_ps(hk)
                    if after_block is not None:
                        for kk in range(k, g.num_blocks):
                            if self.lv[kk][0] == hk:
                                after_block(kk)
                continue
            dz2 = torch.empty_like(a)
            fused_pool = pool == 2 and c.dtype == torch.uint8
            de = torch.empty_like(a) if (pool == 2 and not fused_pool) else None
            if fused_pool:
                with self._t("pool_route_bwd", N, hk, 0.0, self._act_bytes(N, hk, 1 + 0.25 + 1 / 16)):
                    hp.pool_route_bwd(dout, c, sc, dz2, self.slope)
            else:
                with self._t("tail_bwd", N, hk, 0.0, self._act_bytes(N, hk, 4.25 if pool == 2 else 3)):
                    hp.block_tail_bwd(dout, c, xin, sc, dz2, de, pool, self.slope)
            if pool == 1:
                de = dout
            fl = self._conv_flops(N, hk)
            batched = self.x3 and hp.wgrad_x3_supported(N, F_, F_, hk, hk)
            if not batched:
                wws = self._workspace("wgrad", hp.conv3x3_wgrad_ws_bytes(N, F_, F_, hk, hk), dev)
                with self._t("conv3x3_wgrad", N, hk, fl, self._act_bytes(N, hk, 2)):
                    hp.conv3x3_wgrad(a, dz2, G[name + ".conv2.weight"], G[name + ".conv2.bias"], wws)
            dz1 = torch.empty_like(a)
            with self._t("conv3x3_dgrad", N, hk, fl, self._act_bytes(N, hk, 3)):
                hp.conv3x3_dgrad(dz2, self._wpk[name + ".conv2.b"], F_, dz1, act=a, slope=self.slope, x3=self.x3, p16=self.p16)
            if not batched:
                with self._t("conv3x3_wgrad", N, hk, fl, self._act_bytes(N, hk, 2)):
                    hp.conv3x3_wgrad(xin, dz1, G[name + ".conv1.weight"], G[name + ".conv1.bias"], wws)
            dx = torch.empty_like(a) if batched else dz2
            if fused_pool:
                with self._t("conv3x3_dgrad_unpool", N, hk, fl, self._act_bytes(N, hk, 2 + 0.25 + 1 / 16)):
                    hp.conv3x3_dgrad_unpool(dz1, self._wpk[name + ".conv1.b"], F_, dout, c, dx, self.slope, p16=self.p16)
            else:
                with self._t("conv3x3_dgrad", N, hk, fl, self._act_bytes(N, hk, 3)):
                    hp.conv3x3_dgrad(dz1, self._wpk[name + ".conv1.b"], F_, dx, add=de, slope=self.slope, x3=self.x3, p16=self.p16)
            dout = dx
            if batched:
                pending.append((a, dz2, name + ".conv2"))
                pending.append((xin, dz1, name + ".conv1"))
                if k == 0 or self.lv[k - 1][0] != hk:
                    flush(hk)
                    if after_block is not None:
                        for kk in range(k, g.num_blocks):
                            if self.lv[kk][0] == hk:
                                after_block(kk)
            elif after_block is not None:
                after_block(k)
        ws = self._workspace("stem", hp.stem_ws_bytes(N, g.in_ch, F_, g.H, g.W, g.stem_k, g.stem_s, g.stem_p), dev)
        stem_flops = 2.0 * N * F_ * g.in_ch * g.stem_k * g.stem_k * self.h0 * self.h0
        with self._t("stem_wgrad", N, self.h0, stem_flops, 4.0 * N * (g.in_ch * g.H * g.W + F_ * self.h0 * self.h0)):
            stem_x3, stem_p16 = self._stem_wgrad_kind()
            hp.stem_wgrad(x, dout, G["conv1.weight"], G["conv1.bias"], ws, g.stem_k, g.stem_s, g.stem_p, x3=stem_x3, p16=stem_p16)
        if saved.get("ps_scope") is not None:
            saved["ps_scope"].release()
            saved["blocks"] = []


def param_names(num_blocks: int) -> List[str]:
    names = ["conv1.weight", "conv1.bias"]
    for k in range(num_blocks):
        for j in (1, 2):
            names += [f"residual_blocks.{k}.conv{j}.weight", f"residual_blocks.{k}.conv{j}.bias"]
    names += ["out.weight", "out.bias"]
    return names


class ConvStackFn(torch.autograd.Function):

    @staticmethod
    def forward(ctx, engine: ConvStack, masks, names, x, *params):
        P = {n: p.detach() for n, p in zip(names, params)}
        y, saved = engine.forward(x.detach(), P, masks, save=True)
        ctx.engine, ctx.saved, ctx.names, ctx.P = engine, saved, names, P
        return y

    @staticmethod
    def backward(ctx, dy):
        G = {n: torch.empty_like(p) for n, p in ctx.P.items()}
        ctx.engine.backward(ctx.saved, dy, ctx.P, G)
        ctx.saved = None
        return (None, None, None, None) + tuple(G[n] for n in ctx.names)
```

### pytorch-face-detection-from-scratch_amd/csrc/fdet_conv3x3_ps.hip

```cpp
#include "fdet_conv3x3_x3.h"
#include "fdet_ps.h"
#include "fdet_ldsdma.h"
#include <algorithm>

using namespace fdet;

typedef __attribute__((address_space(3))) void* lds_void_t;
typedef const __attribute__((address_space(1))) void* glb_void_t;
typedef unsigned u32x4 __attribute__((ext_vector_type(4)));

namespace {

#ifndef PS_DBG
#define PS_DBG 0
#endif
constexpr int PSA = 9 * 2 * 64;
constexpr int PS_ROWI = 10;

enum { PSE_FWD_FULL = 0, PSE_DGRAD_ACT = 1, PSE_FWD_POOL = 2, PSE_DGRAD_ADDPOOL = 3 };

struct PsConvArgs {
  const bf16x8* x;
  const bf16x8* a_hi;
  const bf16x8* a_lo;
  const float* bias;
  bf16x8* y;
  const bf16x8* aux;
  const float* scale;
  bf16x8* pool_ps;
  float* pool_f32;
  unsigned char* route_out;
  const float* dout;
  const unsigned char* route_in;
  float* dx_f32;
  int Hp, Wp, HPp, WPp, plane_p, img_p;
  int Nimg, last0, Wlast, Wf, Wpf, xo;
  unsigned magic_nimg;
  int N, H, W, HP;
  int nch, ntiles;
  int plane_i, img_i, plane_o, img_o;
  unsigned magic_hp;
  float slope;
};

typedef unsigned u32x2_t __attribute__((ext_vector_type(2)));

__device__ __forceinline__ void ps_keep(const f32x16& v) {
#if defined(__HIP_DEVICE_COMPILE__)
  asm volatile("" ::"v"(v));
#endif
}

__device__ __forceinline__ void ps_acc_read(const f32x16& acc, const int r, float& z) {
#if defined(__HIP_DEVICE_COMPILE__)
  asm("v_accvgpr_read_b32 %0, %1" : "=v"(z) : "a"(acc[r]));
#else
  z = acc[r];
#endif
}

template <int MODE, bool P16>
__device__ __forceinline__ void ps_unit(const f32x16& acc, const int gp, const float (&bza)[4], const float (&bzb)[4],
                                        const u32x2_t (&sg)[2], const float slope, const bool ok, const int ob, const int m,
                                        const int half, const int gstride, const int plane_o_bytes,
                                        const __amdgpu_buffer_rsrc_t yrs) {
  float za[4], zb[4];
#pragma unroll
  for (int i = 0; i < 4; ++i) {
#if defined(__HIP_DEVICE_COMPILE__)
    asm("v_accvgpr_read_b32 %0, %1" : "=v"(za[i]) : "a"(acc[8 * gp + i]));
    asm("v_accvgpr_read_b32 %0, %1" : "=v"(zb[i]) : "a"(acc[8 * gp + 4 + i]));
#else
    za[i] = acc[8 * gp + i]; zb[i] = acc[8 * gp + 4 + i];
#endif
  }
  if (MODE == PSE_FWD_FULL) {
#pragma unroll
    for (int i = 0; i < 4; ++i) {
      const float wa = za[i] + bza[i], wb = zb[i] + bzb[i];
      za[i] = fmaxf(wa, wa * slope);
      zb[i] = fmaxf(wb, wb * slope);
    }
  } else if (MODE == PSE_DGRAD_ACT) {
#pragma unroll
    for (int i = 0; i < 4; ++i) {
      za[i] *= ps_join(sg[0][i >> 1], 0u, i & 1) > 0.f ? 1.f : slope;
      zb[i] *= ps_join(sg[1][i >> 1], 0u, i & 1) > 0.f ? 1.f : slope;
    }
  }
  unsigned ha[2], la[2], hb[2], lb[2];
  if (P16) {
    ps_hi4(za, ha);
    ps_hi4(zb, hb);
  } else {
    ps_split4(za, ha, la);
    ps_split4(zb, hb, lb);
  }
#pragma unroll
  for (int k = 0; k < 2; ++k) {
    auto r1 = __builtin_amdgcn_permlane32_swap(ha[k], hb[k], false, false);
    ha[k] = r1[0]; hb[k] = r1[1];
    if (!P16) {
      auto r2 = __builtin_amdgcn_permlane32_swap(la[k], lb[k], false, false);
      la[k] = r2[0]; lb[k] = r2[1];
    }
  }
  const int G = 4 * m + 2 * gp + half;
  const unsigned off = ok ? (unsigned)(ob + G * gstride) * 16u : 0x80000000u;
  __builtin_amdgcn_raw_buffer_store_b128(u32x4{ha[0], ha[1], hb[0], hb[1]}, yrs, off, 0, 0);
  if (!P16) __builtin_amdgcn_raw_buffer_store_b128(u32x4{la[0], la[1], lb[0], lb[1]}, yrs, off, plane_o_bytes, 0);
}

template <int MODE, int WP, bool P16>
__global__ void __launch_bounds__(256, 1)
k_conv3x3_ps(const PsConvArgs p) {
  constexpr bool WOVEN = MODE == PSE_FWD_FULL || MODE == PSE_DGRAD_ACT || MODE == PSE_DGRAD_ADDPOOL;
  extern __shared__ __attribute__((aligned(16))) char smem[];
  bf16x8* const lds = reinterpret_cast<bf16x8*>(smem);
  const int tid = threadIdx.x, lane = tid & 63;
  const int wid = __builtin_amdgcn_readfirstlane(tid >> 6);
  const int l31 = lane & 31, half = lane >> 5;
  constexpr int WPL = WP == 64 ? 6 : 5, R = 512 / WP, PT = (R + 2) * WP + 8, NBI = (R + 2) * WP / 64;
  constexpr int buf_units = 2 * PSA + 4 * PT;
  const int HP = p.HP;
  int qn[4];
#pragma unroll
  for (int n = 0; n < 4; ++n) qn[n] = WP == 64 ? (2 * wid + (n & 1)) * 64 + (n >> 1) * 32 : (4 * wid + n) * 32;
  constexpr bool POOLM = MODE == PSE_FWD_POOL || MODE == PSE_DGRAD_ADDPOOL;
  if (POOLM) {
#pragma unroll
    for (int n = 0; n < 4; ++n) qn[n] = (WP == 64 ? (2 * wid + (n >> 1)) * 64 : (4 * wid + (n >> 1)) * 32) + (n & 1);
  }
  const int lb = POOLM ? (WP == 64 ? 2 * l31 : 2 * l31 + 32 * (l31 >> 4)) : l31;
  int tile = blockIdx.x, tend = p.ntiles, tstep = gridDim.x;
  if ((gridDim.x & 7) == 0) {
    const int grp = blockIdx.x & 7, chunk = (p.ntiles + 7) >> 3;
    tile = grp * chunk + (blockIdx.x >> 3);
    tend = min((grp + 1) * chunk, p.ntiles);
    tstep = gridDim.x >> 3;
    if (tile >= tend) tile = tend = p.ntiles;
  }
  if (tile >= tend) return;

  unsigned ro[PS_ROWI];
#define PS_ROWOFF(T)                                                                               \
  {                                                                                                \
    const int v0_ = (T) * R;                                                                       \
    _Pragma("unroll") for (int i_ = 0; i_ < PS_ROWI; ++i_) {                                       \
      const int u_ = i_ * 64 + lane;                                                               \
      const int vv_ = v0_ - 1 + (u_ >> WPL) + HP;                                                  \
      const int nn_ = (int)__umulhi((unsigned)vv_, p.magic_hp);                                    \
      ro[i_] = (unsigned)(((PS_DBG & 8) ? 1 : nn_) * p.img_i + (vv_ - nn_ * HP) * WP + (u_ & (WP - 1))) * 16u; \
    }                                                                                              \
  }
  const unsigned lds0 = (unsigned)(size_t)(lds_void_t)smem;
  const dma_u32x4 wrs = dma_rsrc((wid >> 1) ? p.a_lo : p.a_hi, (unsigned)p.nch * PSA * 16u);
  const dma_u32x4 xrs = dma_rsrc(p.x - p.img_i, (unsigned)(p.N + 2) * (unsigned)p.img_i * 16u);
  const unsigned wvoff = (unsigned)((wid & 1) * 576 + lane) * 16u;
#define PS_DMA(C, BS)                                                                              \
  if (!(PS_DBG & 4) && !(P16 && wid >= 2)) {                  \
    const unsigned db_ = lds0 + (unsigned)(BS) * (buf_units * 16);                                 \
    const unsigned ad_ = db_ + (unsigned)((wid >> 1) * PSA + (wid & 1) * 576) * 16u;               \
    _Pragma("unroll") for (int k_ = 0; k_ < ((PS_DBG & 16) ? 0 : 9); ++k_)                          \
      dma_piece(ad_ + k_ * 1024, wvoff, wrs, (unsigned)(C) * (PSA * 16) + k_ * 1024);              \
    const unsigned bso_ = (unsigned)((wid >> 1) * p.plane_i + (2 * (C) + (wid & 1)) * HP * WP) * 16u; \
    const unsigned bd_ = db_ + (unsigned)(2 * PSA + wid * PT) * 16u;                               \
    _Pragma("unroll") for (int i_ = 0; i_ < NBI; ++i_) dma_piece(bd_ + i_ * 1024, ro[i_], xrs, bso_); \
  }

  f32x16 accA[2][4], accB[WOVEN ? 2 : 1][WOVEN ? 4 : 1];
  if (WOVEN) {
#pragma unroll
    for (int m = 0; m < 2; ++m)
#pragma unroll
      for (int n = 0; n < 4; ++n)
#pragma unroll
        for (int r = 0; r < 16; ++r) accB[WOVEN ? m : 0][WOVEN ? n : 0][r] = 0.f;
  }

  float bz[2][4][4];
#pragma unroll
  for (int m = 0; m < 2; ++m)
#pragma unroll
    for (int g = 0; g < 4; ++g)
#pragma unroll
      for (int i = 0; i < 4; ++i) bz[m][g][i] = (MODE == PSE_FWD_FULL || MODE == PSE_FWD_POOL) ? p.bias[32 * m + 8 * g + 4 * half + i] : 0.f;

  const int a_off = half * 64 + l31;
  const int b_off = 2 * PSA + half * PT + lb;
  const int gstride = HP * WP, plane_o_bytes = p.plane_o * 16;
  const __amdgpu_buffer_rsrc_t yrs = __builtin_amdgcn_make_buffer_rsrc(p.y, 0, (int)((size_t)p.N * p.img_o * 16), 0x00020000);

  int ob[4];
  bool okn[4];
#pragma unroll
  for (int n = 0; n < 4; ++n) { ob[n] = 0; okn[n] = false; }
#define PS_GEO(T)                                                                                  \
  {                                                                                                \
    _Pragma("unroll") for (int n_ = 0; n_ < 4; ++n_) {                                             \
      const int q_ = qn[n_] + l31;                                                                 \
      const int col_ = q_ & (WP - 1);                                                              \
      const int v_ = (T) * R + (q_ >> WPL);                                                        \
      const int nn_ = (int)__umulhi((unsigned)v_, p.magic_hp), y_ = v_ - nn_ * HP;                 \
      okn[n_] = nn_ < p.N && y_ < p.H && col_ < (nn_ >= p.last0 ? p.Wlast : p.W);                  \
      ob[n_] = nn_ * p.img_o + y_ * WP + col_ + 1;                                                 \
    }                                                                                              \
  }
  u32x2_t sgp[4][2][2][2];
#pragma unroll
  for (int n = 0; n < 4; ++n)
#pragma unroll
    for (int m = 0; m < 2; ++m)
#pragma unroll
      for (int gp = 0; gp < 2; ++gp) sgp[n][m][gp][0] = sgp[n][m][gp][1] = u32x2_t{0u, 0u};
#define PS_SIGNS()                                                                                 \
  {                                                                                                \
    _Pragma("unroll") for (int n = 0; n < 4; ++n) {                                                \
      const u32x2_t* ap = reinterpret_cast<const u32x2_t*>(p.aux + (okn[n] ? ob[n] : 0)) + half;   \
      _Pragma("unroll") for (int m = 0; m < 2; ++m)                                                \
        _Pragma("unroll") for (int gp = 0; gp < 2; ++gp) {                                         \
          const size_t ga = (size_t)(4 * m + 2 * gp) * gstride, gb = ga + (size_t)gstride;         \
          sgp[n][m][gp][0] = ap[ga * 2];                                                           \
          sgp[n][m][gp][1] = ap[gb * 2];                                                           \
        }                                                                                          \
    }                                                                                              \
  }

  int young = 0;
  int sb = 0;
#define PS_WAITN(K) else if (young == K) asm volatile("s_waitcnt vmcnt(" #K ")" ::: "memory");
#define PS_OPEN()                                                                                  \
  {                                                                                                \
    if (young == 0) asm volatile("s_waitcnt vmcnt(0)" ::: "memory");                               \
    PS_WAITN(4) PS_WAITN(8) PS_WAITN(12) PS_WAITN(16) PS_WAITN(32) PS_WAITN(36) PS_WAITN(40) PS_WAITN(44) PS_WAITN(48) PS_WAITN(63) \
    else asm volatile("s_waitcnt vmcnt(0)" ::: "memory");                                          \
    __builtin_amdgcn_s_barrier();                                                                  \
  }
#define PS_NEXT(C)                                                                                 \
  {                                                                                                \
    if ((C) + 1 < p.nch) {                                                                         \
      PS_DMA((C) + 1, sb ^ 1)                                                                      \
    } else if (tile + tstep < tend) {                                                              \
      PS_ROWOFF(tile + tstep)                                                                      \
      PS_DMA(0, sb ^ 1)                                                                            \
    }                                                                                              \
    __builtin_amdgcn_sched_barrier(0);                                                             \
  }
  bf16x8 ah[2][2], al[2][2], bh[2][4], bl[2][4];
#define PS_FRAGS(F, T)                                                                             \
  {                                                                                                \
    const int to_ = ((T) / 3) * WP + (T) % 3;                                                      \
    _Pragma("unroll") for (int m_ = 0; m_ < 2; ++m_) {                                             \
      ah[F][m_] = Aw[(T) * 128 + m_ * 32];                                                         \
      if (!P16) al[F][m_] = Aw[PSA + (T) * 128 + m_ * 32];                                         \
    }                                                                                              \
    _Pragma("unroll") for (int n_ = 0; n_ < 4; ++n_) {                                             \
      bh[F][n_] = Bw[qn[n_] + to_];                                                                \
      if (!P16) bl[F][n_] = Bw[2 * PT + qn[n_] + to_];                                             \
    }                                                                                              \
  }
#define PS_BODY(ACC, FIRST, JOB, PREV)                                                             \
  {                                                                                                \
    const bf16x8* buf_ = lds + sb * buf_units;                                                     \
    const bf16x8* Aw = buf_ + a_off;                                                               \
    const bf16x8* Bw = buf_ + b_off;                                                               \
    PS_FRAGS(0, 0)                                                                                 \
    __builtin_amdgcn_sched_barrier(0);                                                             \
    _Pragma("unroll") for (int t = 0; t < 9; ++t) {                                                \
      const int F = t & 1;                                                                         \
      if (t < 8) PS_FRAGS(F ^ 1, t + 1)                                                            \
      if (!(PS_DBG & 2)) {                                                                         \
        _Pragma("unroll") for (int m = 0; m < 2; ++m)                                              \
          _Pragma("unroll") for (int n = 0; n < 4; ++n) {                                          \
            const f32x16 zero_ = {};                                                               \
            if (P16) {                                                                             \
              ACC[m][n] = __builtin_amdgcn_mfma_f32_32x32x16_bf16(ah[F][m], bh[F][n], ((FIRST) && t == 0) ? zero_ : ACC[m][n], 0, 0, 0); \
            } else {                                                                               \
              ACC[m][n] = __builtin_amdgcn_mfma_f32_32x32x16_bf16(ah[F][m], bl[F][n], ((FIRST) && t == 0) ? zero_ : ACC[m][n], 0, 0, 0); \
              ACC[m][n] = __builtin_amdgcn_mfma_f32_32x32x16_bf16(al[F][m], bh[F][n], ACC[m][n], 0, 0, 0); \
              ACC[m][n] = __builtin_amdgcn_mfma_f32_32x32x16_bf16(ah[F][m], bh[F][n], ACC[m][n], 0, 0, 0); \
            }                                                                                      \
          }                                                                                        \
      }                                                                                            \
      if ((JOB) != 0 && t < 8 && !(PS_DBG & 1)) {                                                  \
        if constexpr (MODE == PSE_DGRAD_ADDPOOL) {                                                 \
           \
          _Pragma("unroll") for (int e_ = 0; e_ < 2; ++e_) {                                       \
            const int it_ = ((JOB) - 1) * 16 + 2 * t + e_;                                         \
            const int m_ = it_ >> 4, gp_ = (it_ >> 3) & 1, ab_ = (it_ >> 2) & 1, i_ = it_ & 3;     \
            const int arg_ = (int)((rkp[m_][gp_][ab_] >> (8 * i_ + 4)) & 3u);                      \
            const float gv_ = dgp[m_][gp_][ab_][i_];                                               \
            const int so_ = (32 * m_ + 16 * gp_ + 8 * ab_ + i_) * p.H * p.Wf * 4;                  \
            _Pragma("unroll") for (int r_ = 0; r_ < 2; ++r_) {                                     \
              float z0_, z1_;                                                                      \
              ps_acc_read(PREV[WOVEN ? m_ : 0][WOVEN ? 2 * r_ : 0], 8 * gp_ + 4 * ab_ + i_, z0_);  \
              ps_acc_read(PREV[WOVEN ? m_ : 0][WOVEN ? 2 * r_ + 1 : 0], 8 * gp_ + 4 * ab_ + i_, z1_); \
              z0_ += arg_ == 2 * r_ ? gv_ : 0.f;                                                   \
              z1_ += arg_ == 2 * r_ + 1 ? gv_ : 0.f;                                               \
              __builtin_amdgcn_raw_buffer_store_b64(u32x2_t{__builtin_bit_cast(unsigned, z0_), __builtin_bit_cast(unsigned, z1_)}, prs, sto, \
                                                    so_ + r_ * p.Wf * 4, 0);                       \
            }                                                                                      \
          }                                                                                        \
        } else {                                                                                   \
          const int n_ = ((JOB) - 1) * 2 + (t >> 2), m_ = (t >> 1) & 1, gp_ = t & 1;               \
          ps_unit<MODE, P16>(PREV[WOVEN ? m_ : 0][WOVEN ? n_ : 0], gp_, bz[m_][2 * gp_], bz[m_][2 * gp_ + 1], sgp[n_][m_][gp_], p.slope, okn[n_], ob[n_], m_, \
                        half, gstride, plane_o_bytes, yrs);                                        \
        }                                                                                          \
      }                                                                                            \
       \
       \
      if (P16) {    \
        _Pragma("unroll") for (int i = 0; i < 8; ++i) {                                            \
          __builtin_amdgcn_sched_group_barrier(0x008, 1, 0);                                       \
          if (i < 6) __builtin_amdgcn_sched_group_barrier(0x100, 1, 0);                            \
          if ((JOB) != 0) __builtin_amdgcn_sched_group_barrier(0x002, 6, 0);                       \
          if ((JOB) != 0 && (i >= 7 || (MODE == PSE_DGRAD_ADDPOOL && i >= 4))) __builtin_amdgcn_sched_group_barrier(0x040, 1, 0); \
        }                                                                                          \
      } else {                                                                                     \
      _Pragma("unroll") for (int i = 0; i < 12; ++i) {                                             \
        __builtin_amdgcn_sched_group_barrier(0x008, 1, 0);                                         \
        __builtin_amdgcn_sched_group_barrier(0x100, 1, 0);                                         \
        if ((JOB) != 0) __builtin_amdgcn_sched_group_barrier(0x002, 3, 0);                         \
      }                                                                                            \
      _Pragma("unroll") for (int i = 0; i < 12; ++i) {                                             \
        __builtin_amdgcn_sched_group_barrier(0x008, 1, 0);                                         \
        if ((JOB) != 0) __builtin_amdgcn_sched_group_barrier(0x002, 3, 0);                         \
        if ((JOB) != 0 && (i >= 10 || (MODE == PSE_DGRAD_ADDPOOL && i >= 8))) __builtin_amdgcn_sched_group_barrier(0x040, 1, 0); \
      }                                                                                            \
      }                                                                                            \
    }                                                                                              \
    sb ^= 1;                                                                                       \
  }
  const __amdgpu_buffer_rsrc_t prs = __builtin_amdgcn_make_buffer_rsrc(MODE == PSE_FWD_POOL ? (void*)p.pool_ps : (void*)p.dx_f32, 0,
      MODE == PSE_FWD_POOL ? (int)((size_t)p.N * p.img_p * 16) : (int)((size_t)p.Nimg * 64 * p.H * p.Wf * 4), 0x00020000);
  const __amdgpu_buffer_rsrc_t frs = __builtin_amdgcn_make_buffer_rsrc(p.pool_f32, 0, (int)((size_t)p.Nimg * 64 * p.Hp * p.Wpf * 4), 0x00020000);
  const __amdgpu_buffer_rsrc_t rrs = __builtin_amdgcn_make_buffer_rsrc(p.route_out, 0, (int)((size_t)p.N * 64 * p.Hp * p.Wp), 0x00020000);
  const int pool_cnt = MODE == PSE_FWD_POOL ? 4 * ((P16 ? 1 : 2) * (p.pool_ps != nullptr) + (p.route_out != nullptr) + 8 * (p.pool_f32 != nullptr)) : 63;
#define PS_WIN(T)                                                                                  \
    const int rb_ = WP == 64 ? 2 * wid : 4 * wid + 2 * (l31 >> 4);                                 \
    const int v_ = (T) * R + rb_;                                                                  \
    const int nn = (int)__umulhi((unsigned)v_, p.magic_hp), y = v_ - nn * HP;                      \
    const int xp = WP == 64 ? l31 : (l31 & 15), yp = y >> 1;                                       \
    const bool okw = nn < p.N && y < p.H && 2 * xp < (nn >= p.last0 ? p.Wlast : p.W);              \
                \
    const int si = p.last0 == 0 ? 0 : (p.Nimg == 1 ? nn : (int)__umulhi((unsigned)nn, p.magic_nimg)); \
    const int ni = nn - si * p.Nimg, xg = si * (p.xo >> 1) + xp;
  float dgp[2][2][2][4];
  unsigned rkp[2][2][2];
  unsigned sto = 0x80000000u;
#pragma unroll
  for (int m = 0; m < 2; ++m)
#pragma unroll
    for (int gp = 0; gp < 2; ++gp)
#pragma unroll
      for (int ab = 0; ab < 2; ++ab) {
        rkp[m][gp][ab] = 0u;
#pragma unroll
        for (int i = 0; i < 4; ++i) dgp[m][gp][ab][i] = 0.f;
      }
#define PS_POOLPREF(T)                                                                             \
  {                                                                                                \
    PS_WIN(T)                                                                                      \
    const int HWp = p.Hp * p.Wpf, HWr = p.Hp * p.Wp;                                               \
    const int pbase = okw ? (ni * 64 * p.Hp + yp) * p.Wpf + xg : 0;                                \
    const int rbase = okw ? (nn * 8 * p.Hp + yp) * p.Wp + xp : 0;                                  \
    _Pragma("unroll") for (int m = 0; m < 2; ++m)                                                  \
      _Pragma("unroll") for (int gp = 0; gp < 2; ++gp)                                             \
        _Pragma("unroll") for (int ab = 0; ab < 2; ++ab) {                                         \
          const int G = 4 * m + 2 * gp + ab;                                                       \
          _Pragma("unroll") for (int i = 0; i < 4; ++i) {                                          \
            const float v_ = p.dout[pbase + (8 * G + 4 * half + i) * HWp];                         \
            dgp[m][gp][ab][i] = okw ? v_ : 0.f;                                                    \
          }                                                                                        \
          rkp[m][gp][ab] = *reinterpret_cast<const unsigned*>(p.route_in + (size_t)(rbase + G * HWr) * 8 + 4 * half); \
        }                                                                                          \
    sto = okw ? (unsigned)(((ni * 64 + 4 * half) * p.H + y) * p.Wf + 2 * xg) * 4u : 0x80000000u;   \
  }
#define PS_EPI_FWD_POOL(ACC, T)                                                                    \
  if (!(PS_DBG & 1)) {                                                                             \
    PS_WIN(T)                                                                                      \
    const int sb0 = okw ? nn * p.img_i + y * WP + 2 * xp + 1 : 0;                                  \
    u32x2_t sk[2][2][4][4];                                                                        \
    float scv[2][2][2][4];                                                                         \
    _Pragma("unroll") for (int m = 0; m < 2; ++m)                                                  \
      _Pragma("unroll") for (int gp = 0; gp < 2; ++gp) {                                           \
        const size_t ga = (size_t)(4 * m + 2 * gp) * gstride, gb = ga + (size_t)gstride;           \
        _Pragma("unroll") for (int n = 0; n < 4; ++n) {                                            \
          const u32x2_t* ap = reinterpret_cast<const u32x2_t*>(p.aux + sb0 + (n >> 1) * WP + (n & 1)) + half; \
          sk[m][gp][n][0] = ap[ga * 2];                                                            \
          sk[m][gp][n][1] = P16 ? u32x2_t{0u, 0u} : ap[(ga + p.plane_i) * 2];                      \
          sk[m][gp][n][2] = ap[gb * 2];                                                            \
          sk[m][gp][n][3] = P16 ? u32x2_t{0u, 0u} : ap[(gb + p.plane_i) * 2];                      \
        }                                                                                          \
        _Pragma("unroll") for (int i = 0; i < 4; ++i) {                                            \
          const int ch = 32 * m + 16 * gp + 4 * half + i;                                          \
          scv[m][gp][0][i] = (p.scale && okw) ? p.scale[ni * 64 + ch] : 1.f;                       \
          scv[m][gp][1][i] = (p.scale && okw) ? p.scale[ni * 64 + ch + 8] : 1.f;                   \
        }                                                                                          \
      }                                                                                            \
     \
     \
    float pvs[2][2][2][4];                                                                         \
    unsigned rts[2][2][2];                                                                         \
    _Pragma("unroll") for (int m = 0; m < 2; ++m)                                                  \
      _Pragma("unroll") for (int gp = 0; gp < 2; ++gp) {                                           \
        unsigned rt[2] = {0u, 0u};                                                                 \
        _Pragma("unroll") for (int ab = 0; ab < 2; ++ab)                                           \
          _Pragma("unroll") for (int i = 0; i < 4; ++i) {                                          \
            float mx = -INFINITY;                                                                  \
            int arg = 0;                                                                           \
            unsigned bits = 0;                                                                     \
            _Pragma("unroll") for (int n = 0; n < 4; ++n) {                                        \
              float z;                                                                             \
              ps_acc_read(ACC[m][n], 8 * gp + 4 * ab + i, z);                                      \
              const float w_ = z + bz[m][2 * gp + ab][i];                                          \
              z = fmaxf(w_, w_ * p.slope);                                                         \
              bits |= (z > 0.f ? 1u : 0u) << n;                                                    \
              const float u_ = z * scv[m][gp][ab][i] + ps_join(sk[m][gp][n][2 * ab][i >> 1], sk[m][gp][n][2 * ab + 1][i >> 1], i & 1); \
              if (u_ > mx || u_ != u_) { mx = u_; arg = n; }    \
            }                                                                                      \
            pvs[m][gp][ab][i] = mx;                                                                \
            rt[ab] |= (bits | ((unsigned)arg << 4)) << (8 * i);                                    \
          }                                                                                        \
        rts[m][gp][0] = rt[0]; rts[m][gp][1] = rt[1];                                              \
      }                                                                                            \
    if (p.pool_f32) {                 \
      _Pragma("unroll") for (int m = 0; m < 2; ++m)                                                \
        _Pragma("unroll") for (int gp = 0; gp < 2; ++gp) {                                         \
          const unsigned off = okw ? (unsigned)(((ni * 64 + 32 * m + 16 * gp + 4 * half) * p.Hp + yp) * p.Wpf + xg) * 4u : 0x80000000u; \
          _Pragma("unroll") for (int jj = 0; jj < 8; ++jj)                                         \
            __builtin_amdgcn_raw_buffer_store_b32(__builtin_bit_cast(unsigned, pvs[m][gp][jj >> 2][jj & 3]), frs, off, \
                                                  (8 * (jj >> 2) + (jj & 3)) * p.Hp * p.Wpf * 4, 0); \
        }                                                                                          \
    }                                                                                              \
     \
    _Pragma("unroll") for (int m = 0; m < 2; ++m)                                                  \
      _Pragma("unroll") for (int gp = 0; gp < 2; ++gp) {                                           \
        _Pragma("unroll") for (int i = 0; i < 4; ++i) {                                            \
          auto r_ = __builtin_amdgcn_permlane32_swap(__float_as_uint(pvs[m][gp][0][i]), __float_as_uint(pvs[m][gp][1][i]), false, false); \
          const unsigned r0_ = r_[0], r1_ = r_[1];    \
          pvs[m][gp][0][i] = __uint_as_float(r0_); pvs[m][gp][1][i] = __uint_as_float(r1_);        \
        }                                                                                          \
        { auto r_ = __builtin_amdgcn_permlane32_swap(rts[m][gp][0], rts[m][gp][1], false, false); rts[m][gp][0] = r_[0]; rts[m][gp][1] = r_[1]; } \
      }                                                                                            \
    if (p.pool_ps) {                                                                               \
      _Pragma("unroll") for (int m = 0; m < 2; ++m)                                                \
        _Pragma("unroll") for (int gp = 0; gp < 2; ++gp) {                                         \
          const int G = 4 * m + 2 * gp + half;                                                     \
          unsigned ha[2], la[2], hb[2], lb2[2];                                                    \
          if (P16) { ps_hi4(pvs[m][gp][0], ha); ps_hi4(pvs[m][gp][1], hb); }                       \
          else { ps_split4(pvs[m][gp][0], ha, la); ps_split4(pvs[m][gp][1], hb, lb2); }            \
          const unsigned off = okw ? (unsigned)(nn * p.img_p + (G * p.HPp + yp) * p.WPp + xp + 1) * 16u : 0x80000000u; \
          __builtin_amdgcn_raw_buffer_store_b128(u32x4{ha[0], ha[1], hb[0], hb[1]}, prs, off, 0, 0); \
          if (!P16) __builtin_amdgcn_raw_buffer_store_b128(u32x4{la[0], la[1], lb2[0], lb2[1]}, prs, off, p.plane_p * 16, 0); \
        }                                                                                          \
    }                                                                                              \
    if (p.route_out) {                                                                             \
      _Pragma("unroll") for (int m = 0; m < 2; ++m)                                                \
        _Pragma("unroll") for (int gp = 0; gp < 2; ++gp) {                                         \
          const int G = 4 * m + 2 * gp + half;                                                     \
          const unsigned off = okw ? (unsigned)(((nn * 8 + G) * p.Hp + yp) * p.Wp + xp) * 8u : 0x80000000u; \
          __builtin_amdgcn_raw_buffer_store_b64(u32x2_t{rts[m][gp][0], rts[m][gp][1]}, rrs, off, 0, 0); \
        }                                                                                          \
    }                                                                                              \
  } else {                                                                                         \
    _Pragma("unroll") for (int m = 0; m < 2; ++m)                                                  \
      _Pragma("unroll") for (int n = 0; n < 4; ++n) ps_keep(ACC[m][n]);                            \
  }
#define PS_EPI_ADDPOOL(ACC, T)                                                                     \
  if (!(PS_DBG & 1)) {                                                                             \
    PS_WIN(T)                                                                                      \
    float dg[2][2][2][4];                                                                          \
    unsigned rk[2][2][2];                                                                          \
    const int HWp = p.Hp * p.Wpf;                                                                  \
    const int pbase = okw ? (ni * 64 * p.Hp + yp) * p.Wpf + xg : 0;                                \
    _Pragma("unroll") for (int m = 0; m < 2; ++m)                                                  \
      _Pragma("unroll") for (int gp = 0; gp < 2; ++gp)                                             \
        _Pragma("unroll") for (int ab = 0; ab < 2; ++ab) {                                         \
          const int G = 4 * m + 2 * gp + ab;                                                       \
          _Pragma("unroll") for (int i = 0; i < 4; ++i) dg[m][gp][ab][i] = okw ? p.dout[pbase + (8 * G + 4 * half + i) * HWp] : 0.f; \
          rk[m][gp][ab] = okw ? *reinterpret_cast<const unsigned*>(p.route_in + (size_t)(((nn * 8 + G) * p.Hp + yp) * p.Wp + xp) * 8 + 4 * half) : 0u; \
        }                                                                                          \
    _Pragma("unroll") for (int m = 0; m < 2; ++m)                                                  \
      _Pragma("unroll") for (int gp = 0; gp < 2; ++gp)                                             \
        _Pragma("unroll") for (int ab = 0; ab < 2; ++ab)                                           \
          _Pragma("unroll") for (int i = 0; i < 4; ++i) {                                          \
            const int ch = 32 * m + 16 * gp + 8 * ab + 4 * half + i;                               \
            const int arg = (int)((rk[m][gp][ab] >> (8 * i + 4)) & 3u);                            \
            const float gv = dg[m][gp][ab][i];                                                     \
            _Pragma("unroll") for (int r = 0; r < 2; ++r) {                                        \
              float z0, z1;                                                                        \
              ps_acc_read(ACC[m][2 * r], 8 * gp + 4 * ab + i, z0);                                 \
              ps_acc_read(ACC[m][2 * r + 1], 8 * gp + 4 * ab + i, z1);                             \
              z0 += arg == 2 * r ? gv : 0.f;                                                       \
              z1 += arg == 2 * r + 1 ? gv : 0.f;                                                   \
              const unsigned off = okw ? (unsigned)(((ni * 64 + ch) * p.H + y + r) * p.Wf + 2 * xg) * 4u : 0x80000000u; \
              __builtin_amdgcn_raw_buffer_store_b64(u32x2_t{__builtin_bit_cast(unsigned, z0), __builtin_bit_cast(unsigned, z1)}, prs, off, 0, 0); \
            }                                                                                      \
          }                                                                                        \
  } else {                                                                                         \
    _Pragma("unroll") for (int m = 0; m < 2; ++m)                                                  \
      _Pragma("unroll") for (int n = 0; n < 4; ++n) ps_keep(ACC[m][n]);                            \
  }
#define PS_EPILOGUE(ACC)                                                                           \
  if constexpr (MODE == PSE_FWD_POOL) { PS_EPI_FWD_POOL(ACC, etile) }                              \
  else if constexpr (MODE == PSE_DGRAD_ADDPOOL) { PS_EPI_ADDPOOL(ACC, etile) }                     \
  else if (!(PS_DBG & 1)) {                                                                        \
    if (MODE == PSE_DGRAD_ACT) PS_SIGNS()                                                          \
    _Pragma("unroll") for (int n = 0; n < 4; ++n)                                                  \
      _Pragma("unroll") for (int m = 0; m < 2; ++m)                                                \
        _Pragma("unroll") for (int gp = 0; gp < 2; ++gp)                                           \
          ps_unit<MODE, P16>(ACC[m][n], gp, bz[m][2 * gp], bz[m][2 * gp + 1], sgp[n][m][gp], p.slope,  \
                        okn[n], ob[n], m, half, gstride, plane_o_bytes, yrs);                      \
  } else {                                                                                         \
    _Pragma("unroll") for (int m = 0; m < 2; ++m)                                                  \
      _Pragma("unroll") for (int n = 0; n < 4; ++n) ps_keep(ACC[m][n]);                            \
  }
#define PS_TILE(ACC, PREV)                                                                         \
  {                                                                                                \
    PS_OPEN()                                                                                      \
    PS_NEXT(0)                                                                                     \
    PS_BODY(ACC, 1, (WOVEN ? 1 : 0), PREV)                                                         \
    young = (WOVEN && !(PS_DBG & 1)) ? (MODE == PSE_DGRAD_ADDPOOL ? 32 : (P16 ? 8 : 16)) : 0;      \
    PS_OPEN()                                                                                      \
    PS_NEXT(1)                                                                                     \
    PS_BODY(ACC, 0, (WOVEN ? 2 : 0), PREV)                                                         \
    for (int c = 2; c < p.nch; ++c) {                                                              \
      PS_OPEN()                                                                                    \
      PS_NEXT(c)                                                                                   \
      PS_BODY(ACC, 0, 0, PREV)                                                                     \
      young = 0;                                                                                   \
    }                                                                                              \
    PS_GEO(tile)                                                                                   \
    etile = tile;                                                                                  \
    if (WOVEN && MODE == PSE_DGRAD_ACT && !(PS_DBG & 1)) {                                         \
      PS_SIGNS()                                                                                   \
      young += 32;                                                                                 \
    }                                                                                              \
    if constexpr (MODE == PSE_DGRAD_ADDPOOL) {                                                     \
      if (!(PS_DBG & 1)) {                                                                         \
        PS_POOLPREF(tile)                                                                          \
        young = min(young + 40, 63);                                                               \
      }                                                                                            \
    }                                                                                              \
    if (!WOVEN) {                                                                                  \
      PS_EPILOGUE(ACC)                                                                             \
      young = (PS_DBG & 1) ? 0 : (POOLM ? pool_cnt : 32);                                          \
    }                                                                                              \
  }

  int etile = tile;
  PS_ROWOFF(tile)
  PS_DMA(0, 0)
  if (WOVEN) {
    for (;;) {
      PS_TILE(accA, accB)
      tile += tstep;
      if (tile >= tend) { PS_EPILOGUE(accA) break; }
      PS_TILE(accB, accA)
      tile += tstep;
      if (tile >= tend) { PS_EPILOGUE(accB) break; }
    }
  } else {
    for (; tile < tend; tile += tstep) PS_TILE(accA, accA)
  }
#undef PS_TILE
#undef PS_EPILOGUE
#undef PS_EPI_ADDPOOL
#undef PS_EPI_FWD_POOL
#undef PS_POOLPREF
#undef PS_WIN
#undef PS_WAITN
#undef PS_BODY
#undef PS_FRAGS
#undef PS_NEXT
#undef PS_OPEN
#undef PS_GEO
#undef PS_SIGNS
#undef PS_DMA
#undef PS_ROWOFF
}

#ifndef PS_TU
#define PS_TU (-1)
#endif
#define PS_CAT_(a, b) a##b
#define PS_CAT(a, b) PS_CAT_(a, b)
#define PS_TU_NAME PS_CAT(fdet_ps_launch_, PS_TU)
template <int MODE, int WP, bool P16>
int launch_ps(const PsConvArgs& p, size_t lds, int grid, hipStream_t st) {
  static bool attr_set = false;
  constexpr int lds_max = 2 * (2 * PSA + 4 * 648) * 16;
  if (!attr_set) {
    if ((int)lds > lds_max || hipFuncSetAttribute((const void*)k_conv3x3_ps<MODE, WP, P16>, hipFuncAttributeMaxDynamicSharedMemorySize, lds_max) != hipSuccess) {
      (void)hipGetLastError();
      return fail(FDET_ELAUNCH, "conv3x3_ps: cannot reserve %zu bytes of LDS", lds);
    }
    attr_set = true;
  }
  hipLaunchKernelGGL((k_conv3x3_ps<MODE, WP, P16>), dim3(grid), dim3(256), lds, st, p);
  return check_launch("fdet_conv3x3_ps");
}

}
#define PS_DECL_LAUNCH(N) extern "C" int fdet_ps_launch_##N(const void* args, size_t lds, int grid, void* stream);
PS_DECL_LAUNCH(0) PS_DECL_LAUNCH(1) PS_DECL_LAUNCH(2) PS_DECL_LAUNCH(3) PS_DECL_LAUNCH(4) PS_DECL_LAUNCH(5) PS_DECL_LAUNCH(6) PS_DECL_LAUNCH(7)
PS_DECL_LAUNCH(8) PS_DECL_LAUNCH(9) PS_DECL_LAUNCH(10) PS_DECL_LAUNCH(11) PS_DECL_LAUNCH(12) PS_DECL_LAUNCH(13) PS_DECL_LAUNCH(14) PS_DECL_LAUNCH(15)
#if PS_TU >= 0
extern "C" int PS_TU_NAME(const void* args, size_t lds, int grid, void* stream) {
  return launch_ps<(PS_TU & 7) / 2, (PS_TU & 1) ? 64 : 32, (PS_TU >= 8)>(*reinterpret_cast<const PsConvArgs*>(args), lds, grid, (hipStream_t)stream);
}
#endif
namespace {
#if PS_TU == -1
typedef int (*ps_launch_fn)(const void*, size_t, int, void*);
const ps_launch_fn PS_LAUNCHERS[16] = {fdet_ps_launch_0, fdet_ps_launch_1, fdet_ps_launch_2, fdet_ps_launch_3,
                                       fdet_ps_launch_4, fdet_ps_launch_5, fdet_ps_launch_6, fdet_ps_launch_7,
                                       fdet_ps_launch_8, fdet_ps_launch_9, fdet_ps_launch_10, fdet_ps_launch_11,
                                       fdet_ps_launch_12, fdet_ps_launch_13, fdet_ps_launch_14, fdet_ps_launch_15};
struct PsPoolIO {
  const float* scale = nullptr; void* pool_ps = nullptr; float* pool_f32 = nullptr; unsigned char* route_out = nullptr;
  const float* dout = nullptr; const unsigned char* route_in = nullptr; float* dx_f32 = nullptr;
};

const char* ps_conv_refusal(int pooled, int N, int Cin, int Cout, int H, int W) {
  PsGeo gi, go, gp;
  PsStrips sp, spo;
  if (!(Cout == 64 && Cin % 16 == 0 && Cin >= 32)) return "Cout must be 64 and Cin a multiple of 16, at least 32";
  if (!(ps_geo_strips(N, Cin, H, W, gi, sp) && ps_geo_strips(N, Cout, H, W, go, spo) && gi.WP >= 32 && sp.Ws + 2 <= gi.WP))
    return "unsupported map (W + 2 <= 32 or 64 slots, or an even width in strips)";
  if (!((size_t)(gi.N + 2) * gi.img * 16 < ((size_t)1 << 32) && (size_t)(go.N + 2) * go.img * 16 < ((size_t)1 << 32)))
    return "tensor too large for the 32-bit byte offsets of the DMA descriptors";
  if (pooled) {
    if ((H & 1) || (W & 1) || Cin != 64) return "pooled block: even map and 64 channels required";
    if ((size_t)N * 64 * H * W * 4 >= ((size_t)1 << 31)) return "pooled block: tensor too large for 32-bit offsets";
    if (pooled == 2 && sp.S != 1) return "a strip map writes its pooled output as fp32 NCHW (pool_f32)";
    if (pooled == 2 && !ps_geo(gi.N, 64, H / 2, W / 2, gp)) return "the pooled map has no PS layout";
  }
  if ((long)gi.N * gi.HP + gi.HP >= (1 << 20)) return "too many rows";
  return nullptr;
}

int run_ps(int mode, const void* x, const void* wpk, const float* bias, const void* aux, void* y, const PsPoolIO& io, int N,
           int Cin, int Cout, int H, int W, float slope, hipStream_t st, bool p16 = false) {
  PsGeo gi, gp;
  PsStrips sp;
  const bool pooled = mode == PSE_FWD_POOL || mode == PSE_DGRAD_ADDPOOL;
  FDET_REQUIRE(x && wpk && (y || pooled), "conv3x3_ps: null pointer");
  const int pool_mode = !pooled ? 0 : (mode == PSE_FWD_POOL && io.pool_ps ? 2 : 1);
  if (const char* why = ps_conv_refusal(pool_mode, N, Cin, Cout, H, W))
    return fail(FDET_EINVAL, "conv3x3_ps: %s (N=%d Cin=%d Cout=%d H=%d W=%d)", why, N, Cin, Cout, H, W);
  ps_geo_strips(N, Cin, H, W, gi, sp);
  const int Nimg = N, Wfull = W;
  N = gi.N; W = sp.Ws;
  FDET_REQUIRE(slope >= 0.f && slope <= 1.f, "conv3x3_ps: slope must be in [0, 1]");
  PsConvArgs p;
  p.x = reinterpret_cast<const bf16x8*>(x);
  const size_t units = (size_t)(Cin / 16) * PSA;
  p.a_hi = reinterpret_cast<const bf16x8*>(wpk);
  p.a_lo = p.a_hi + units;
  p.bias = bias;
  p.y = reinterpret_cast<bf16x8*>(y);
  p.aux = reinterpret_cast<const bf16x8*>(aux);
  p.scale = io.scale; p.pool_ps = reinterpret_cast<bf16x8*>(io.pool_ps); p.pool_f32 = io.pool_f32; p.route_out = io.route_out;
  p.dout = io.dout; p.route_in = io.route_in; p.dx_f32 = io.dx_f32;
  p.Hp = H / 2; p.Wp = W / 2; p.HPp = p.WPp = p.plane_p = p.img_p = 0;
  p.Nimg = Nimg; p.last0 = sp.S > 1 ? (sp.S - 1) * Nimg : 0; p.Wlast = sp.Wlast; p.Wf = Wfull; p.Wpf = Wfull / 2; p.xo = sp.Ws;
  p.magic_nimg = Nimg > 1 ? magic_of(Nimg) : 0u;
  PsGeo go;
  PsStrips spo;
  ps_geo_strips(Nimg, Cout, H, Wfull, go, spo);
  if (pool_mode == 2) {
    ps_geo(N, 64, H / 2, W / 2, gp);
    p.HPp = gp.HP; p.WPp = gp.WP; p.plane_p = gp.plane; p.img_p = gp.img;
  }
  p.N = N; p.H = H; p.W = W; p.HP = gi.HP;
  p.nch = Cin / 16;
  const int R = 512 / gi.WP, PT = (R + 2) * gi.WP + 8;
  const long vr = (long)N * gi.HP;
  p.ntiles = (int)((vr + R - 1) / R);
  p.plane_i = gi.plane; p.img_i = gi.img; p.plane_o = go.plane; p.img_o = go.img;
  p.magic_hp = magic_of(gi.HP);
  p.slope = slope;
  const size_t lds = (size_t)2 * (2 * PSA + 4 * PT) * 16;
  const int grid = std::min(p.ntiles, num_cus());
  const bool w64 = gi.WP == 64;
  switch (mode) {
    case PSE_FWD_FULL:
      FDET_REQUIRE(bias, "conv3x3_ps_fwd: bias is required");
      break;
    case PSE_DGRAD_ACT:
      FDET_REQUIRE(aux, "conv3x3_ps_dgrad_act: the activation is required");
      break;
    case PSE_FWD_POOL:
      FDET_REQUIRE(bias && aux && (io.pool_ps || io.pool_f32), "conv3x3_ps_fwd_pool: bias, skip and an output are required");
      break;
    default:
      FDET_REQUIRE(io.dout && io.route_in && io.dx_f32, "conv3x3_ps_dgrad_unpool: dout, route and dx are required");
      break;
  }
  return PS_LAUNCHERS[(p16 ? 8 : 0) + 2 * mode + (w64 ? 1 : 0)](&p, lds, grid, (void*)st);
}
#endif

}

#if PS_TU == -1
extern "C" int fdet_conv3x3_ps_ok(int N, int Cin, int Cout, int H, int W, int pooled) {
  return ps_conv_refusal(pooled, N, Cin, Cout, H, W) == nullptr;
}

extern "C" int fdet_conv3x3_ps_fwd(const void* x_ps, const void* wpk, const float* bias, void* y_ps, int N, int Cin,
                                   int Cout, int H, int W, float slope, void* stream) {
  return run_ps(PSE_FWD_FULL, x_ps, wpk, bias, nullptr, y_ps, PsPoolIO{}, N, Cin, Cout, H, W, slope, (hipStream_t)stream);
}

extern "C" int fdet_conv3x3_ps_dgrad_act(const void* dz_ps, const void* wpk, const void* act_ps, void* dx_ps, int N,
                                         int Cin, int Cout, int H, int W, float slope, void* stream) {
  return run_ps(PSE_DGRAD_ACT, dz_ps, wpk, nullptr, act_ps, dx_ps, PsPoolIO{}, N, Cout, Cin, H, W, slope, (hipStream_t)stream);
}

extern "C" int fdet_conv3x3_ps_fwd_pool(const void* x_ps, const void* wpk, const float* bias, const void* skip_ps,
                                        const float* drop_scale, void* pool_ps, float* pool_f32, unsigned char* route8,
                                        int N, int Cin, int Cout, int H, int W, float slope, void* stream) {
  PsPoolIO io;
  io.scale = drop_scale; io.pool_ps = pool_ps; io.pool_f32 = pool_f32; io.route_out = route8;
  return run_ps(PSE_FWD_POOL, x_ps, wpk, bias, skip_ps, nullptr, io, N, Cin, Cout, H, W, slope, (hipStream_t)stream);
}

extern "C" int fdet_conv3x3_ps_dgrad_unpool(const void* dz_ps, const void* wpk, const float* dout_pooled,
                                            const unsigned char* route8, float* dx, int N, int Cin, int Cout, int H, int W,
                                            float slope, void* stream) {
  PsPoolIO io;
  io.dout = dout_pooled; io.route_in = route8; io.dx_f32 = dx;
  return run_ps(PSE_DGRAD_ADDPOOL, dz_ps, wpk, nullptr, nullptr, nullptr, io, N, Cout, Cin, H, W, slope, (hipStream_t)stream);
}

extern "C" int fdet_conv3x3_ps_fwd_p16(const void* x_ps, const void* wpk, const float* bias, void* y_ps, int N, int Cin,
                                       int Cout, int H, int W, float slope, void* stream) {
  return run_ps(PSE_FWD_FULL, x_ps, wpk, bias, nullptr, y_ps, PsPoolIO{}, N, Cin, Cout, H, W, slope, (hipStream_t)stream, true);
}
extern "C" int fdet_conv3x3_ps_dgrad_act_p16(const void* dz_ps, const void* wpk, const void* act_ps, void* dx_ps, int N,
                                             int Cin, int Cout, int H, int W, float slope, void* stream) {
  return run_ps(PSE_DGRAD_ACT, dz_ps, wpk, nullptr, act_ps, dx_ps, PsPoolIO{}, N, Cout, Cin, H, W, slope, (hipStream_t)stream, true);
}
extern "C" int fdet_conv3x3_ps_fwd_pool_p16(const void* x_ps, const void* wpk, const float* bias, const void* skip_ps,
                                            const float* drop_scale, void* pool_ps, float* pool_f32, unsigned char* route8,
                                            int N, int Cin, int Cout, int H, int W, float slope, void* stream) {
  PsPoolIO io;
  io.scale = drop_scale; io.pool_ps = pool_ps; io.pool_f32 = pool_f32; io.route_out = route8;
  return run_ps(PSE_FWD_POOL, x_ps, wpk, bias, skip_ps, nullptr, io, N, Cin, Cout, H, W, slope, (hipStream_t)stream, true);
}
extern "C" int fdet_conv3x3_ps_dgrad_unpool_p16(const void* dz_ps, const void* wpk, const float* dout_pooled,
                                                const unsigned char* route8, float* dx, int N, int Cin, int Cout, int H, int W,
                                                float slope, void* stream) {
  PsPoolIO io;
  io.dout = dout_pooled; io.route_in = route8; io.dx_f32 = dx;
  return run_ps(PSE_DGRAD_ADDPOOL, dz_ps, wpk, nullptr, nullptr, nullptr, io, N, Cout, Cin, H, W, slope, (hipStream_t)stream, true);
}

#endif
```

### pytorch-face-detection-from-scratch_amd/ps.py

```python
from __future__ import annotations

import functools

import torch

from ._native import FdetError, check, lib, ptr, stream

F32 = torch.float32


@functools.lru_cache(maxsize=None)
def strips_of(W: int):
    S = int(lib().fdet_ps_strips(int(W)))
    if S <= 1:
        return S, (W if S == 1 else 0)
    return S, ((W + S - 1) // S + 1) & ~1


class PsTensor:

    def __init__(self, N: int, C: int, H: int, W: int, device):
        nbytes = int(lib().fdet_ps_bytes(N, C, H, W))
        if nbytes == 0:
            raise FdetError(f"PsTensor: unsupported shape ({N},{C},{H},{W}) (C % 8 == 0; W <= 63 or even)")
        self.shape = (N, C, H, W)
        self.strips = strips_of(W)[0]
        self.buf = torch.zeros(nbytes // 4, dtype=F32, device=device)
        self._off = int(lib().fdet_ps_image0_offset(N, C, H, W))

    @property
    def data(self) -> int:
        return ptr(self.buf) + self._off

    @property
    def device(self):
        return self.buf.device

    @classmethod
    def from_f32(cls, x: torch.Tensor, out: "PsTensor" = None) -> "PsTensor":
        if x.dim() != 4 or x.dtype != F32 or not x.is_contiguous():
            raise TypeError("PsTensor.from_f32: expected a contiguous fp32 (N,C,H,W) tensor")
        N, C, H, W = x.shape
        t = out if out is not None else cls(N, C, H, W, x.device)
        if t.shape != (N, C, H, W):
            raise ValueError(f"PsTensor.from_f32: buffer is {t.shape}, tensor is {tuple(x.shape)}")
        check(lib().fdet_ps_from_f32(ptr(x), t.data, N, C, H, W, stream()), "fdet_ps_from_f32")
        return t

    def to_f32(self, out: torch.Tensor = None) -> torch.Tensor:
        N, C, H, W = self.shape
        y = out if out is not None else torch.empty(N, C, H, W, dtype=F32, device=self.device)
        if tuple(y.shape) != self.shape:
            raise ValueError("PsTensor.to_f32: output shape mismatch")
        check(lib().fdet_ps_to_f32(self.data, ptr(y), N, C, H, W, stream()), "fdet_ps_to_f32")
        return y


def halo_exchange(t: PsTensor, zero_only: bool = False, p16: bool = False) -> None:
    if t.strips <= 1:
        return
    N, C, H, W = t.shape
    check(lib().fdet_ps_halo_exchange(t.data, N, C, H, W, int(zero_only), int(p16), stream()), "fdet_ps_halo_exchange")


def route8_shape(N: int, C: int, H: int, W: int):
    S, Ws = strips_of(W)
    return (N * S, C // 8, H // 2, Ws // 2, 8)


def _same(a: PsTensor, shape, name):
    if not isinstance(a, PsTensor) or a.shape != tuple(shape):
        raise ValueError(f"{name}: expected a PsTensor of shape {tuple(shape)}, got {getattr(a, 'shape', type(a))}")


def _fn(name: str, p16: bool):
    return getattr(lib(), name + "_p16" if p16 else name)


def conv3x3_ps_fwd(x: PsTensor, wpk: torch.Tensor, bias: torch.Tensor, y: PsTensor, slope: float = 0.2, p16: bool = False) -> None:
    N, cin, H, W = x.shape
    cout = int(bias.shape[0])
    _same(y, (N, cout, H, W), "conv3x3_ps_fwd: y")
    if wpk.numel() != cout * cin * 9:
        raise ValueError("conv3x3_ps_fwd: packed weight size does not match (Cout,Cin)")
    check(_fn("fdet_conv3x3_ps_fwd", p16)(x.data, ptr(wpk), ptr(bias), y.data, N, cin, cout, H, W, float(slope), stream()),
          "fdet_conv3x3_ps_fwd")


def conv3x3_ps_dgrad_act(dz: PsTensor, wpk_bwd: torch.Tensor, act: PsTensor, dx: PsTensor, slope: float = 0.2, p16: bool = False) -> None:
    N, cout, H, W = dz.shape
    cin = dx.shape[1]
    _same(dx, (N, cin, H, W), "conv3x3_ps_dgrad_act: dx")
    _same(act, (N, cin, H, W), "conv3x3_ps_dgrad_act: act")
    if wpk_bwd.numel() != cout * cin * 9:
        raise ValueError("conv3x3_ps_dgrad_act: packed weight size does not match (Cout,Cin)")
    check(_fn("fdet_conv3x3_ps_dgrad_act", p16)(dz.data, ptr(wpk_bwd), act.data, dx.data, N, cin, cout, H, W, float(slope),
                                                stream()), "fdet_conv3x3_ps_dgrad_act")


def conv3x3_ps_ok(N: int, Cin: int, Cout: int, H: int, W: int, pooled: int = 0) -> bool:
    return bool(lib().fdet_conv3x3_ps_ok(int(N), int(Cin), int(Cout), int(H), int(W), int(pooled)))


def conv3x3_wgrad_ps_ws_bytes(L: int, N: int, C: int, H: int, W: int) -> int:
    return int(lib().fdet_conv3x3_wgrad_ps_ws_bytes(L, N, C, H, W))


def conv3x3_wgrad_ps_batched(xs, dzs, dWs, dbs, ws: torch.Tensor, p16: bool = False) -> None:
    import ctypes
    L = len(xs)
    N, C, H, W = xs[0].shape
    for x, dz, dW, db in zip(xs, dzs, dWs, dbs):
        _same(x, (N, C, H, W), "conv3x3_wgrad_ps: x")
        _same(dz, (N, C, H, W), "conv3x3_wgrad_ps: dz")
        if tuple(dW.shape) != (C, C, 3, 3) or tuple(db.shape) != (C,):
            raise ValueError("conv3x3_wgrad_ps: dW / db shapes")
    arr = ctypes.c_void_p * L
    check(_fn("fdet_conv3x3_wgrad_ps_batched", p16)(arr(*[x.data for x in xs]), arr(*[z.data for z in dzs]),
                                                    arr(*[ptr(t) for t in dWs]), arr(*[ptr(t) for t in dbs]), L, N, C, H, W,
                                                    ptr(ws), ws.numel() * 4, stream()), "fdet_conv3x3_wgrad_ps_batched")


def route8_like(N: int, C: int, H: int, W: int, device) -> torch.Tensor:
    return torch.empty(*route8_shape(N, C, H, W), dtype=torch.uint8, device=device)


def conv3x3_ps_fwd_pool(x: PsTensor, wpk, bias, skip: PsTensor, drop_scale, pool_ps: PsTensor = None,
                        pool_f32: torch.Tensor = None, route8: torch.Tensor = None, slope: float = 0.2, p16: bool = False) -> None:
    N, cin, H, W = x.shape
    cout = int(bias.shape[0])
    _same(skip, (N, cout, H, W), "conv3x3_ps_fwd_pool: skip")
    if pool_ps is not None:
        _same(pool_ps, (N, cout, H // 2, W // 2), "conv3x3_ps_fwd_pool: pool_ps")
    if pool_f32 is not None and tuple(pool_f32.shape) != (N, cout, H // 2, W // 2):
        raise ValueError("conv3x3_ps_fwd_pool: pool_f32 shape")
    if route8 is not None and tuple(route8.shape) != route8_shape(N, cout, H, W):
        raise ValueError("conv3x3_ps_fwd_pool: route8 shape")
    if pool_ps is not None and x.strips > 1:
        raise ValueError("conv3x3_ps_fwd_pool: a strip map writes its pooled output as fp32 NCHW (pool_f32)")
    if drop_scale is not None and tuple(drop_scale.shape) != (N, cout):
        raise ValueError("conv3x3_ps_fwd_pool: drop_scale shape")
    if wpk.numel() != cout * cin * 9:
        raise ValueError("conv3x3_ps_fwd_pool: packed weight size does not match (Cout,Cin)")
    check(_fn("fdet_conv3x3_ps_fwd_pool", p16)(x.data, ptr(wpk), ptr(bias), skip.data, ptr(drop_scale),
                                               pool_ps.data if pool_ps is not None else None, ptr(pool_f32),
                                               ptr(route8, torch.uint8), N, cin, cout, H, W, float(slope), stream()),
          "fdet_conv3x3_ps_fwd_pool")


def pool_route_bwd_ps(dout_pooled: torch.Tensor, route8: torch.Tensor, drop_scale, dz2: PsTensor, slope: float = 0.2,
                      p16: bool = False) -> None:
    N, C, H, W = dz2.shape
    if tuple(dout_pooled.shape) != (N, C, H // 2, W // 2) or tuple(route8.shape) != route8_shape(N, C, H, W):
        raise ValueError("pool_route_bwd_ps: shapes")
    check(_fn("fdet_pool_route_bwd_ps", p16)(ptr(dout_pooled), ptr(route8, torch.uint8), ptr(drop_scale), dz2.data, N, C, H, W,
                                             float(slope), stream()), "fdet_pool_route_bwd_ps")


def conv3x3_ps_dgrad_unpool(dz: PsTensor, wpk_bwd, dout_pooled: torch.Tensor, route8: torch.Tensor, dx: torch.Tensor,
                            slope: float = 0.2, p16: bool = False) -> None:
    N, cout, H, W = dz.shape
    cin = dx.shape[1]
    if tuple(dx.shape) != (N, cin, H, W) or tuple(dout_pooled.shape) != (N, cin, H // 2, W // 2) or \
            tuple(route8.shape) != route8_shape(N, cin, H, W):
        raise ValueError("conv3x3_ps_dgrad_unpool: shapes")
    if wpk_bwd.numel() != cout * cin * 9:
        raise ValueError("conv3x3_ps_dgrad_unpool: packed weight size does not match (Cout,Cin)")
    check(_fn("fdet_conv3x3_ps_dgrad_unpool", p16)(dz.data, ptr(wpk_bwd), ptr(dout_pooled), ptr(route8, torch.uint8), ptr(dx),
                                                   N, cin, cout, H, W, float(slope), stream()), "fdet_conv3x3_ps_dgrad_unpool")


def stem_fwd_ps(x: torch.Tensor, w: torch.Tensor, bias: torch.Tensor, y: PsTensor, k: int, stride: int, pad: int,
                p16: bool = False) -> None:
    N, cin, H, W = x.shape
    F_ = int(w.shape[0])
    Ho, Wo = (H + 2 * pad - k) // stride + 1, (W + 2 * pad - k) // stride + 1
    _same(y, (N, F_, Ho, Wo), "stem_fwd_ps: y")
    if x.dtype == torch.uint8:
        if not x.is_contiguous():
            raise ValueError("stem_fwd_ps: uint8 frames must be contiguous")
        check(lib().fdet_stem_fwd_ps_u8(ptr(x, torch.uint8), ptr(w), ptr(bias), y.data, N, cin, F_, H, W, k, stride, pad, int(p16), stream()),
              "fdet_stem_fwd_ps_u8")
        return
    check(_fn("fdet_stem_fwd_ps", p16)(ptr(x), ptr(w), ptr(bias), y.data, N, cin, F_, H, W, k, stride, pad, stream()), "fdet_stem_fwd_ps")


def _ps_ptr_array(ts):
    import ctypes
    if ts is None:
        return None
    return (ctypes.c_void_p * len(ts))(*[(t.data if t is not None else None) for t in ts])


def block_chain_fwd_ps(x, wpk1, b1, wpk2, b2, scales, a_ps, c_ps, out_ps, out_last: torch.Tensor, slope: float = 0.2,
                       p16: bool = False) -> None:
    from .hotpath import _ptr_array
    nb = len(wpk1)
    N, C, H, W = out_last.shape
    x_is_ps = isinstance(x, PsTensor)
    if x_is_ps:
        _same(x, (N, C, H, W), "block_chain_fwd_ps: x")
    elif tuple(x.shape) != (N, C, H, W) or x.dtype != F32 or not x.is_contiguous():
        raise ValueError("block_chain_fwd_ps: x must be a PsTensor or a contiguous fp32 tensor of the output's shape")
    if not (len(b1) == len(wpk2) == len(b2) == nb) or (scales is not None and len(scales) != nb):
        raise ValueError("block_chain_fwd_ps: inconsistent per-block lists")
    for lst, n_, nm in ((a_ps, nb, "a"), (c_ps, nb, "c"), (out_ps, nb - 1, "out")):
        if lst is not None:
            if len(lst) != n_:
                raise ValueError(f"block_chain_fwd_ps: {nm} needs {n_} entries")
            for t in lst:
                if t is not None:
                    _same(t, (N, C, H, W), "block_chain_fwd_ps: " + nm)
    check(_fn("fdet_block_chain_fwd_ps", p16)(x.data if x_is_ps else ptr(x), int(x_is_ps), _ptr_array(wpk1), _ptr_array(b1),
                                        _ptr_array(wpk2), _ptr_array(b2), _ptr_array(scales), _ps_ptr_array(a_ps),
                                        _ps_ptr_array(c_ps), _ps_ptr_array(out_ps), ptr(out_last), nb, N, C, H, W,
                                        float(slope), stream()), "fdet_block_chain_fwd_ps")


def block_chain_bwd_ps(dout: torch.Tensor, wpk1b, wpk2b, scales, a_ps, c_ps, dz1_ps, dz2_ps, dx: torch.Tensor,
                       slope: float = 0.2, p16: bool = False) -> None:
    from .hotpath import _ptr_array
    nb = len(wpk1b)
    N, C, H, W = dout.shape
    if not (len(wpk2b) == len(a_ps) == len(c_ps) == len(dz1_ps) == len(dz2_ps) == nb):
        raise ValueError("block_chain_bwd_ps: inconsistent per-block lists")
    for lst, nm in ((a_ps, "a"), (c_ps, "c"), (dz1_ps, "dz1"), (dz2_ps, "dz2")):
        for t in lst:
            _same(t, (N, C, H, W), "block_chain_bwd_ps: " + nm)
    if tuple(dx.shape) != (N, C, H, W):
        raise ValueError("block_chain_bwd_ps: dx shape mismatch")
    check(_fn("fdet_block_chain_bwd_ps", p16)(ptr(dout), _ptr_array(wpk1b), _ptr_array(wpk2b), _ptr_array(scales),
                                        _ps_ptr_array(a_ps), _ps_ptr_array(c_ps), _ps_ptr_array(dz1_ps),
                                        _ps_ptr_array(dz2_ps), ptr(dx), nb, N, C, H, W, float(slope), stream()),
          "fdet_block_chain_bwd_ps")
```

Measured before the change: 92940.

## Emit a packed activation sign bitmask in forward and use it in dgrad

The forward 3x3 conv kernel now also writes a 1-bit-per-element sign mask of its leaky-ReLU output into a separate buffer. The backward dgrad_act kernel reads that mask instead of re-reading the full bf16 activation tensor to decide between slope and 1. This cuts backward activation traffic to a small fraction, at the cost of an extra mask write and extra VALU work in the forward epilogue, plus retuned scheduling groups and wait counts. Mask correctness depends on the mask-offset geometry matching the strip layout.

Result: no change. 93330 (median of 6 runs) (+0.4%).

```diff
diff --git a/include/fdet.h b/include/fdet.h
--- a/include/fdet.h
+++ b/include/fdet.h
@@ -152,6 +152,11 @@
                         int H, int W, float slope, void* stream);
 int fdet_conv3x3_ps_dgrad_act(const void* dz_ps, const void* wpk, const void* act_ps, void* dx_ps, int N, int Cin,
                               int Cout, int H, int W, float slope, void* stream);
+size_t fdet_ps_mask_bytes(int N, int H, int W);
+int fdet_conv3x3_ps_fwd_m(const void* x_ps, const void* wpk, const float* bias, void* y_ps, void* mask, int N, int Cin,
+                          int Cout, int H, int W, float slope, void* stream);
+int fdet_conv3x3_ps_dgrad_act_m(const void* dz_ps, const void* wpk, const void* act_ps, const void* mask, void* dx_ps, int N,
+                                int Cin, int Cout, int H, int W, float slope, void* stream);
 
 int fdet_conv3x3_ps_fwd_pool(const void* x_ps, const void* wpk, const float* bias, const void* skip_ps,
                              const float* drop_scale, void* pool_ps, float* pool_f32, unsigned char* route8, int N, int Cin,
@@ -219,6 +224,10 @@
                             int Cout, int H, int W, float slope, void* stream);
 int fdet_conv3x3_ps_dgrad_act_p16(const void* dz_ps, const void* wpk, const void* act_ps, void* dx_ps, int N,
                                   int Cin, int Cout, int H, int W, float slope, void* stream);
+int fdet_conv3x3_ps_fwd_m_p16(const void* x_ps, const void* wpk, const float* bias, void* y_ps, void* mask, int N, int Cin,
+                              int Cout, int H, int W, float slope, void* stream);
+int fdet_conv3x3_ps_dgrad_act_m_p16(const void* dz_ps, const void* wpk, const void* act_ps, const void* mask, void* dx_ps,
+                                    int N, int Cin, int Cout, int H, int W, float slope, void* stream);
 int fdet_conv3x3_ps_fwd_pool_p16(const void* x_ps, const void* wpk, const float* bias, const void* skip_ps,
                                  const float* drop_scale, void* pool_ps, float* pool_f32, unsigned char* route8,
                                  int N, int Cin, int Cout, int H, int W, float slope, void* stream);
diff --git a/pytorch-face-detection-from-scratch_amd/_native.py b/pytorch-face-detection-from-scratch_amd/_native.py
--- a/pytorch-face-detection-from-scratch_amd/_native.py
+++ b/pytorch-face-detection-from-scratch_amd/_native.py
@@ -78,6 +78,9 @@
     "fdet_ps_halo_exchange": (_I, [_P, _I, _I, _I, _I, _I, _I, _P]),
     "fdet_conv3x3_ps_fwd": (_I, [_P, _P, _P, _P, _I, _I, _I, _I, _I, _F, _P]),
     "fdet_conv3x3_ps_dgrad_act": (_I, [_P, _P, _P, _P, _I, _I, _I, _I, _I, _F, _P]),
+    "fdet_ps_mask_bytes": (_SZ, [_I, _I, _I]),
+    "fdet_conv3x3_ps_fwd_m": (_I, [_P, _P, _P, _P, _P, _I, _I, _I, _I, _I, _F, _P]),
+    "fdet_conv3x3_ps_dgrad_act_m": (_I, [_P, _P, _P, _P, _P, _I, _I, _I, _I, _I, _F, _P]),
     "fdet_conv3x3_ps_fwd_pool": (_I, [_P, _P, _P, _P, _P, _P, _P, _P, _I, _I, _I, _I, _I, _F, _P]),
     "fdet_pool_route_bwd_ps": (_I, [_P, _P, _P, _P, _I, _I, _I, _I, _F, _P]),
     "fdet_conv3x3_ps_dgrad_unpool": (_I, [_P, _P, _P, _P, _P, _I, _I, _I, _I, _I, _F, _P]),
@@ -125,6 +128,8 @@
     "fdet_head_bwd": (_I, [_P, _P, _P, _P, _P, _P, _P, _P, _P, _SZ, _I, _I, _I, _I, _I, _I, _P]),
     "fdet_conv3x3_ps_fwd_p16": (_I, [_P, _P, _P, _P, _I, _I, _I, _I, _I, _F, _P]),
     "fdet_conv3x3_ps_dgrad_act_p16": (_I, [_P, _P, _P, _P, _I, _I, _I, _I, _I, _F, _P]),
+    "fdet_conv3x3_ps_fwd_m_p16": (_I, [_P, _P, _P, _P, _P, _I, _I, _I, _I, _I, _F, _P]),
+    "fdet_conv3x3_ps_dgrad_act_m_p16": (_I, [_P, _P, _P, _P, _P, _I, _I, _I, _I, _I, _F, _P]),
     "fdet_conv3x3_ps_fwd_pool_p16": (_I, [_P, _P, _P, _P, _P, _P, _P, _P, _I, _I, _I, _I, _I, _F, _P]),
     "fdet_conv3x3_ps_dgrad_unpool_p16": (_I, [_P, _P, _P, _P, _P, _I, _I, _I, _I, _I, _F, _P]),
     "fdet_pool_route_bwd_ps_p16": (_I, [_P, _P, _P, _P, _I, _I, _I, _I, _F, _P]),
diff --git a/pytorch-face-detection-from-scratch_amd/convstack.py b/pytorch-face-detection-from-scratch_amd/convstack.py
--- a/pytorch-face-detection-from-scratch_amd/convstack.py
+++ b/pytorch-face-detection-from-scratch_amd/convstack.py
@@ -128,6 +128,7 @@
         self.ps = self.pool_fusion and geo.filters == 64 and os.environ.get("FDET_PS", "1") != "0"
         self._ps_pool: Dict[tuple, list] = {}
         self.ps_strips = self.ps and os.environ.get("FDET_PS_STRIPS", "1") != "0"
+        self.signmask = self.ps and os.environ.get("FDET_SIGNMASK", "1") != "0"
         self.p16 = self.x3 and want == "bf16"
         self._cur_N = 1
         self.head_fused = self.x3 and os.environ.get("FDET_HEAD_FUSED", "1") != "0"
@@ -236,6 +237,13 @@
         key = (N, C, H, W, str(dev))
         free = self._ps_pool.setdefault(key, [])
         t = free.pop() if free else psm.PsTensor(N, C, H, W, dev)
+        scope.append((key, t))
+        return t
+
+    def _mask_take(self, scope: "_PsScope", N: int, H: int, W: int, dev) -> "psm.PsMask":
+        key = ("mask", N, H, W, str(dev))
+        free = self._ps_pool.setdefault(key, [])
+        t = free.pop() if free else psm.PsMask(N, H, W, dev)
         scope.append((key, t))
         return t
 
@@ -295,8 +303,10 @@
                 if h_ps is None:
                     h_ps = psm.PsTensor.from_f32(h, out=self._ps_take(scope, N, F_, hk, hk, dev))
                 a_ps = self._ps_take(scope, N, F_, hk, hk, dev)
-                with self._t("conv3x3_fwd", N, hk, self._conv_flops(N, hk), self._act_bytes(N, hk, 2)):
-                    psm.conv3x3_ps_fwd(h_ps, self._wpk[name + ".conv1.f"], P[name + ".conv1.bias"], a_ps, self.slope, p16=self.p16)
+                a_mask = self._mask_take(scope, N, hk, hk, dev) if save and self.signmask else None
+                with self._t("conv3x3_fwd", N, hk, self._conv_flops(N, hk), self._act_bytes(N, hk, 2 + (1 / 32 if a_mask is not None else 0))):
+                    psm.conv3x3_ps_fwd(h_ps, self._wpk[name + ".conv1.f"], P[name + ".conv1.bias"], a_ps, self.slope, p16=self.p16,
+                                       mask=a_mask)
                     psm.halo_exchange(a_ps, p16=self.p16)
                 nxt = (self._ps_block(k + 1) or self._ps_chain(k + 1)) and not self._strips(hk)
                 out_ps = self._ps_take(scope, N, F_, hk // 2, hk // 2, dev) if nxt else None
@@ -307,6 +317,8 @@
                                             route, self.slope, p16=self.p16)
                 if save:
                     saved["blocks"].append((h_ps, a_ps, route))
+                    if a_mask is not None:
+                        saved.setdefault("signs", {})[k] = (a_ps, a_mask)
                 h, h_ps = out, out_ps
                 continue
             run = self._chain_run(k)
@@ -546,6 +558,9 @@
                     xin = psm.PsTensor.from_f32(xin.to(F32).contiguous(), out=self._ps_take(scope, N, F_, hk, hk, dev))
                 if not isinstance(a, psm.PsTensor):
                     a = psm.PsTensor.from_f32(a.to(F32).contiguous(), out=self._ps_take(scope, N, F_, hk, hk, dev))
+                sg_a, a_mask = saved.get("signs", {}).get(k, (None, None))
+                if sg_a is not a:
+                    a_mask = None
                 strips = self._strips(hk)
                 if c.dim() == 4:
                     if strips:
@@ -565,8 +580,8 @@
                 if strips:
                     wgrad_now(a, dz2, name + ".conv2", clean=True)
                 dz1 = self._ps_take(scope, N, F_, hk, hk, dev)
-                with self._t("conv3x3_dgrad", N, hk, fl, self._act_bytes(N, hk, 3)):
-                    psm.conv3x3_ps_dgrad_act(dz2, self._wpk[name + ".conv2.b"], a, dz1, self.slope, p16=self.p16)
+                with self._t("conv3x3_dgrad", N, hk, fl, self._act_bytes(N, hk, 2 + (1 / 32 if a_mask is not None else 0.5))):
+                    psm.conv3x3_ps_dgrad_act(dz2, self._wpk[name + ".conv2.b"], a, dz1, self.slope, p16=self.p16, mask=a_mask)
                 if strips:
                     wgrad_now(xin, dz1, name + ".conv1")
                 dx = torch.empty(N, F_, hk, hk, dtype=F32, device=dev)
diff --git a/pytorch-face-detection-from-scratch_amd/csrc/fdet_conv3x3_ps.hip b/pytorch-face-detection-from-scratch_amd/csrc/fdet_conv3x3_ps.hip
--- a/pytorch-face-detection-from-scratch_amd/csrc/fdet_conv3x3_ps.hip
+++ b/pytorch-face-detection-from-scratch_amd/csrc/fdet_conv3x3_ps.hip
@@ -11,13 +11,20 @@
 
 namespace {
 
+#ifndef PS_VG
+#define PS_VG 4
+#endif
+#ifndef PS_VG16
+#define PS_VG16 8
+#endif
 #ifndef PS_DBG
 #define PS_DBG 0
 #endif
 constexpr int PSA = 9 * 2 * 64;
 constexpr int PS_ROWI = 10;
 
-enum { PSE_FWD_FULL = 0, PSE_DGRAD_ACT = 1, PSE_FWD_POOL = 2, PSE_DGRAD_ADDPOOL = 3 };
+enum { PSE_FWD_FULL = 0, PSE_DGRAD_ACT = 1, PSE_FWD_POOL = 2, PSE_DGRAD_ADDPOOL = 3,
+       PSE_DGRAD_ACT_M = 4 };
 
 struct PsConvArgs {
   const bf16x8* x;
@@ -26,6 +33,7 @@
   const float* bias;
   bf16x8* y;
   const bf16x8* aux;
+  unsigned* mask;
   const float* scale;
   bf16x8* pool_ps;
   float* pool_f32;
@@ -63,7 +71,8 @@
 __device__ __forceinline__ void ps_unit(const f32x16& acc, const int gp, const float (&bza)[4], const float (&bzb)[4],
                                         const u32x2_t (&sg)[2], const float slope, const bool ok, const int ob, const int m,
                                         const int half, const int gstride, const int plane_o_bytes,
-                                        const __amdgpu_buffer_rsrc_t yrs) {
+                                        const __amdgpu_buffer_rsrc_t yrs, unsigned& mk, const unsigned moff,
+                                        const __amdgpu_buffer_rsrc_t mrs) {
   float za[4], zb[4];
 #pragma unroll
   for (int i = 0; i < 4; ++i) {
@@ -86,6 +95,12 @@
     for (int i = 0; i < 4; ++i) {
       za[i] *= ps_join(sg[0][i >> 1], 0u, i & 1) > 0.f ? 1.f : slope;
       zb[i] *= ps_join(sg[1][i >> 1], 0u, i & 1) > 0.f ? 1.f : slope;
+    }
+  } else if (MODE == PSE_DGRAD_ACT_M) {
+#pragma unroll
+    for (int i = 0; i < 4; ++i) {
+      za[i] *= (mk & (1u << (16 * m + 8 * gp + i))) ? 1.f : slope;
+      zb[i] *= (mk & (1u << (16 * m + 8 * gp + 4 + i))) ? 1.f : slope;
     }
   }
   unsigned ha[2], la[2], hb[2], lb[2];
@@ -96,6 +111,14 @@
     ps_split4(za, ha, la);
     ps_split4(zb, hb, lb);
   }
+  if (MODE == PSE_FWD_FULL) {
+    const float tiny = __builtin_bit_cast(float, 0x00008000u);
+    unsigned by = 0u;
+#pragma unroll
+    for (int e = 7; e >= 0; --e) by = by + by + ((e < 4 ? za[e & 3] : zb[e & 3]) > tiny ? 1u : 0u);
+    const unsigned bits = by << (16 * m + 8 * gp);
+    mk = (m | gp) ? (mk | bits) : bits;
+  }
 #pragma unroll
   for (int k = 0; k < 2; ++k) {
     auto r1 = __builtin_amdgcn_permlane32_swap(ha[k], hb[k], false, false);
@@ -109,12 +132,15 @@
   const unsigned off = ok ? (unsigned)(ob + G * gstride) * 16u : 0x80000000u;
   __builtin_amdgcn_raw_buffer_store_b128(u32x4{ha[0], ha[1], hb[0], hb[1]}, yrs, off, 0, 0);
   if (!P16) __builtin_amdgcn_raw_buffer_store_b128(u32x4{la[0], la[1], lb[0], lb[1]}, yrs, off, plane_o_bytes, 0);
+  if (MODE == PSE_FWD_FULL && m == 1 && gp == 1) __builtin_amdgcn_raw_buffer_store_b32(mk, mrs, ok ? moff : 0x80000000u, 0, 0);
 }
 
 template <int MODE, int WP, bool P16>
 __global__ void __launch_bounds__(256, 1)
 k_conv3x3_ps(const PsConvArgs p) {
-  constexpr bool WOVEN = MODE == PSE_FWD_FULL || MODE == PSE_DGRAD_ACT || MODE == PSE_DGRAD_ADDPOOL;
+  constexpr bool DACT = MODE == PSE_DGRAD_ACT || MODE == PSE_DGRAD_ACT_M, DMASK = MODE == PSE_DGRAD_ACT_M;
+  constexpr bool WOVEN = MODE == PSE_FWD_FULL || DACT || MODE == PSE_DGRAD_ADDPOOL;
+  constexpr bool MASKU = MODE == PSE_FWD_FULL || DMASK;
   extern __shared__ __attribute__((aligned(16))) char smem[];
   bf16x8* const lds = reinterpret_cast<bf16x8*>(smem);
   const int tid = threadIdx.x, lane = tid & 63;
@@ -193,8 +219,11 @@
 
   int ob[4];
   bool okn[4];
-#pragma unroll
-  for (int n = 0; n < 4; ++n) { ob[n] = 0; okn[n] = false; }
+  unsigned mo[4], mkw[4];
+  const __amdgpu_buffer_rsrc_t mrs = __builtin_amdgcn_make_buffer_rsrc(p.mask, 0,
+      (MODE == PSE_FWD_FULL && p.mask) ? (int)((size_t)p.N * HP * WP * 8) : 0, 0x00020000);
+#pragma unroll
+  for (int n = 0; n < 4; ++n) { ob[n] = 0; okn[n] = false; mo[n] = 0u; mkw[n] = 0u; }
 #define PS_GEO(T)                                                                                  \
   {                                                                                                \
     _Pragma("unroll") for (int n_ = 0; n_ < 4; ++n_) {                                             \
@@ -204,6 +233,7 @@
       const int nn_ = (int)__umulhi((unsigned)v_, p.magic_hp), y_ = v_ - nn_ * HP;                 \
       okn[n_] = nn_ < p.N && y_ < p.H && col_ < (nn_ >= p.last0 ? p.Wlast : p.W);                  \
       ob[n_] = nn_ * p.img_o + y_ * WP + col_ + 1;                                                 \
+      mo[n_] = (unsigned)((T) * 512 + q_ + 1) * 8u + 4u * half;                                    \
     }                                                                                              \
   }
   u32x2_t sgp[4][2][2][2];
@@ -215,6 +245,9 @@
       for (int gp = 0; gp < 2; ++gp) sgp[n][m][gp][0] = sgp[n][m][gp][1] = u32x2_t{0u, 0u};
 #define PS_SIGNS()                                                                                 \
   {                                                                                                \
+  if constexpr (DMASK) {                                              \
+    _Pragma("unroll") for (int n = 0; n < 4; ++n) mkw[n] = p.mask[okn[n] ? mo[n] >> 2 : 0];        \
+  } else {                                                                                         \
     _Pragma("unroll") for (int n = 0; n < 4; ++n) {                                                \
       const u32x2_t* ap = reinterpret_cast<const u32x2_t*>(p.aux + (okn[n] ? ob[n] : 0)) + half;   \
       _Pragma("unroll") for (int m = 0; m < 2; ++m)                                                \
@@ -224,6 +257,7 @@
           sgp[n][m][gp][1] = ap[gb * 2];                                                           \
         }                                                                                          \
     }                                                                                              \
+  }                                                                                                \
   }
 
   int young = 0;
@@ -232,7 +266,7 @@
 #define PS_OPEN()                                                                                  \
   {                                                                                                \
     if (young == 0) asm volatile("s_waitcnt vmcnt(0)" ::: "memory");                               \
-    PS_WAITN(4) PS_WAITN(8) PS_WAITN(12) PS_WAITN(16) PS_WAITN(32) PS_WAITN(36) PS_WAITN(40) PS_WAITN(44) PS_WAITN(48) PS_WAITN(63) \
+    PS_WAITN(4) PS_WAITN(8) PS_WAITN(10) PS_WAITN(12) PS_WAITN(16) PS_WAITN(18) PS_WAITN(20) PS_WAITN(32) PS_WAITN(36) PS_WAITN(40) PS_WAITN(44) PS_WAITN(48) PS_WAITN(63) \
     else asm volatile("s_waitcnt vmcnt(0)" ::: "memory");                                          \
     __builtin_amdgcn_s_barrier();                                                                  \
   }
@@ -304,7 +338,7 @@
         } else {                                                                                   \
           const int n_ = ((JOB) - 1) * 2 + (t >> 2), m_ = (t >> 1) & 1, gp_ = t & 1;               \
           ps_unit<MODE, P16>(PREV[WOVEN ? m_ : 0][WOVEN ? n_ : 0], gp_, bz[m_][2 * gp_], bz[m_][2 * gp_ + 1], sgp[n_][m_][gp_], p.slope, okn[n_], ob[n_], m_, \
-                        half, gstride, plane_o_bytes, yrs);                                        \
+                        half, gstride, plane_o_bytes, yrs, mkw[n_], mo[n_], mrs);                  \
         }                                                                                          \
       }                                                                                            \
        \
@@ -313,19 +347,21 @@
         _Pragma("unroll") for (int i = 0; i < 8; ++i) {                                            \
           __builtin_amdgcn_sched_group_barrier(0x008, 1, 0);                                       \
           if (i < 6) __builtin_amdgcn_sched_group_barrier(0x100, 1, 0);                            \
-          if ((JOB) != 0) __builtin_amdgcn_sched_group_barrier(0x002, 6, 0);                       \
+          if ((JOB) != 0) __builtin_amdgcn_sched_group_barrier(0x002, MASKU ? PS_VG16 : 6, 0);     \
           if ((JOB) != 0 && (i >= 7 || (MODE == PSE_DGRAD_ADDPOOL && i >= 4))) __builtin_amdgcn_sched_group_barrier(0x040, 1, 0); \
+          if ((JOB) != 0 && MODE == PSE_FWD_FULL && (t & 3) == 3 && i == 7) __builtin_amdgcn_sched_group_barrier(0x040, 1, 0); \
         }                                                                                          \
       } else {                                                                                     \
       _Pragma("unroll") for (int i = 0; i < 12; ++i) {                                             \
         __builtin_amdgcn_sched_group_barrier(0x008, 1, 0);                                         \
         __builtin_amdgcn_sched_group_barrier(0x100, 1, 0);                                         \
-        if ((JOB) != 0) __builtin_amdgcn_sched_group_barrier(0x002, 3, 0);                         \
+        if ((JOB) != 0) __builtin_amdgcn_sched_group_barrier(0x002, MASKU ? PS_VG : 3, 0);         \
       }                                                                                            \
       _Pragma("unroll") for (int i = 0; i < 12; ++i) {                                             \
         __builtin_amdgcn_sched_group_barrier(0x008, 1, 0);                                         \
-        if ((JOB) != 0) __builtin_amdgcn_sched_group_barrier(0x002, 3, 0);                         \
+        if ((JOB) != 0) __builtin_amdgcn_sched_group_barrier(0x002, MASKU ? PS_VG : 3, 0);         \
         if ((JOB) != 0 && (i >= 10 || (MODE == PSE_DGRAD_ADDPOOL && i >= 8))) __builtin_amdgcn_sched_group_barrier(0x040, 1, 0); \
+        if ((JOB) != 0 && MODE == PSE_FWD_FULL && (t & 3) == 3 && i == 11) __builtin_amdgcn_sched_group_barrier(0x040, 1, 0); \
       }                                                                                            \
       }                                                                                            \
     }                                                                                              \
@@ -506,12 +542,12 @@
   if constexpr (MODE == PSE_FWD_POOL) { PS_EPI_FWD_POOL(ACC, etile) }                              \
   else if constexpr (MODE == PSE_DGRAD_ADDPOOL) { PS_EPI_ADDPOOL(ACC, etile) }                     \
   else if (!(PS_DBG & 1)) {                                                                        \
-    if (MODE == PSE_DGRAD_ACT) PS_SIGNS()                                                          \
+    if (DACT) PS_SIGNS()                                                                           \
     _Pragma("unroll") for (int n = 0; n < 4; ++n)                                                  \
       _Pragma("unroll") for (int m = 0; m < 2; ++m)                                                \
         _Pragma("unroll") for (int gp = 0; gp < 2; ++gp)                                           \
           ps_unit<MODE, P16>(ACC[m][n], gp, bz[m][2 * gp], bz[m][2 * gp + 1], sgp[n][m][gp], p.slope,  \
-                        okn[n], ob[n], m, half, gstride, plane_o_bytes, yrs);                      \
+                        okn[n], ob[n], m, half, gstride, plane_o_bytes, yrs, mkw[n], mo[n], mrs);  \
   } else {                                                                                         \
     _Pragma("unroll") for (int m = 0; m < 2; ++m)                                                  \
       _Pragma("unroll") for (int n = 0; n < 4; ++n) ps_keep(ACC[m][n]);                            \
@@ -521,7 +557,8 @@
     PS_OPEN()                                                                                      \
     PS_NEXT(0)                                                                                     \
     PS_BODY(ACC, 1, (WOVEN ? 1 : 0), PREV)                                                         \
-    young = (WOVEN && !(PS_DBG & 1)) ? (MODE == PSE_DGRAD_ADDPOOL ? 32 : (P16 ? 8 : 16)) : 0;      \
+                      \
+    young = (WOVEN && !(PS_DBG & 1)) ? (MODE == PSE_DGRAD_ADDPOOL ? 32 : (P16 ? 8 : 16) + (MODE == PSE_FWD_FULL ? 2 : 0)) : 0; \
     PS_OPEN()                                                                                      \
     PS_NEXT(1)                                                                                     \
     PS_BODY(ACC, 0, (WOVEN ? 2 : 0), PREV)                                                         \
@@ -533,9 +570,9 @@
     }                                                                                              \
     PS_GEO(tile)                                                                                   \
     etile = tile;                                                                                  \
-    if (WOVEN && MODE == PSE_DGRAD_ACT && !(PS_DBG & 1)) {                                         \
+    if (WOVEN && DACT && !(PS_DBG & 1)) {                                                          \
       PS_SIGNS()                                                                                   \
-      young += 32;                                                                                 \
+      young += DMASK ? 4 : 32;                                                                     \
     }                                                                                              \
     if constexpr (MODE == PSE_DGRAD_ADDPOOL) {                                                     \
       if (!(PS_DBG & 1)) {                                                                         \
@@ -606,18 +643,21 @@
 #define PS_DECL_LAUNCH(N) extern "C" int fdet_ps_launch_##N(const void* args, size_t lds, int grid, void* stream);
 PS_DECL_LAUNCH(0) PS_DECL_LAUNCH(1) PS_DECL_LAUNCH(2) PS_DECL_LAUNCH(3) PS_DECL_LAUNCH(4) PS_DECL_LAUNCH(5) PS_DECL_LAUNCH(6) PS_DECL_LAUNCH(7)
 PS_DECL_LAUNCH(8) PS_DECL_LAUNCH(9) PS_DECL_LAUNCH(10) PS_DECL_LAUNCH(11) PS_DECL_LAUNCH(12) PS_DECL_LAUNCH(13) PS_DECL_LAUNCH(14) PS_DECL_LAUNCH(15)
+PS_DECL_LAUNCH(16) PS_DECL_LAUNCH(17) PS_DECL_LAUNCH(18) PS_DECL_LAUNCH(19)
 #if PS_TU >= 0
 extern "C" int PS_TU_NAME(const void* args, size_t lds, int grid, void* stream) {
-  return launch_ps<(PS_TU & 7) / 2, (PS_TU & 1) ? 64 : 32, (PS_TU >= 8)>(*reinterpret_cast<const PsConvArgs*>(args), lds, grid, (hipStream_t)stream);
+  return launch_ps<(PS_TU < 16 ? (PS_TU & 7) / 2 : (int)PSE_DGRAD_ACT_M), (PS_TU & 1) ? 64 : 32, (PS_TU < 16 ? PS_TU >= 8 : PS_TU >= 18)>(
+      *reinterpret_cast<const PsConvArgs*>(args), lds, grid, (hipStream_t)stream);
 }
 #endif
 namespace {
 #if PS_TU == -1
 typedef int (*ps_launch_fn)(const void*, size_t, int, void*);
-const ps_launch_fn PS_LAUNCHERS[16] = {fdet_ps_launch_0, fdet_ps_launch_1, fdet_ps_launch_2, fdet_ps_launch_3,
+const ps_launch_fn PS_LAUNCHERS[20] = {fdet_ps_launch_0, fdet_ps_launch_1, fdet_ps_launch_2, fdet_ps_launch_3,
                                        fdet_ps_launch_4, fdet_ps_launch_5, fdet_ps_launch_6, fdet_ps_launch_7,
                                        fdet_ps_launch_8, fdet_ps_launch_9, fdet_ps_launch_10, fdet_ps_launch_11,
-                                       fdet_ps_launch_12, fdet_ps_launch_13, fdet_ps_launch_14, fdet_ps_launch_15};
+                                       fdet_ps_launch_12, fdet_ps_launch_13, fdet_ps_launch_14, fdet_ps_launch_15,
+                                       fdet_ps_launch_16, fdet_ps_launch_17, fdet_ps_launch_18, fdet_ps_launch_19};
 struct PsPoolIO {
   const float* scale = nullptr; void* pool_ps = nullptr; float* pool_f32 = nullptr; unsigned char* route_out = nullptr;
   const float* dout = nullptr; const unsigned char* route_in = nullptr; float* dx_f32 = nullptr;
@@ -642,7 +682,7 @@
 }
 
 int run_ps(int mode, const void* x, const void* wpk, const float* bias, const void* aux, void* y, const PsPoolIO& io, int N,
-           int Cin, int Cout, int H, int W, float slope, hipStream_t st, bool p16 = false) {
+           int Cin, int Cout, int H, int W, float slope, hipStream_t st, bool p16 = false, void* mask = nullptr) {
   PsGeo gi, gp;
   PsStrips sp;
   const bool pooled = mode == PSE_FWD_POOL || mode == PSE_DGRAD_ADDPOOL;
@@ -662,6 +702,7 @@
   p.bias = bias;
   p.y = reinterpret_cast<bf16x8*>(y);
   p.aux = reinterpret_cast<const bf16x8*>(aux);
+  p.mask = reinterpret_cast<unsigned*>(mask);
   p.scale = io.scale; p.pool_ps = reinterpret_cast<bf16x8*>(io.pool_ps); p.pool_f32 = io.pool_f32; p.route_out = io.route_out;
   p.dout = io.dout; p.route_in = io.route_in; p.dx_f32 = io.dx_f32;
   p.Hp = H / 2; p.Wp = W / 2; p.HPp = p.WPp = p.plane_p = p.img_p = 0;
@@ -690,7 +731,7 @@
       FDET_REQUIRE(bias, "conv3x3_ps_fwd: bias is required");
       break;
     case PSE_DGRAD_ACT:
-      FDET_REQUIRE(aux, "conv3x3_ps_dgrad_act: the activation is required");
+      FDET_REQUIRE(aux || mask, "conv3x3_ps_dgrad_act: the activation or its sign mask is required");
       break;
     case PSE_FWD_POOL:
       FDET_REQUIRE(bias && aux && (io.pool_ps || io.pool_f32), "conv3x3_ps_fwd_pool: bias, skip and an output are required");
@@ -699,6 +740,7 @@
       FDET_REQUIRE(io.dout && io.route_in && io.dx_f32, "conv3x3_ps_dgrad_unpool: dout, route and dx are required");
       break;
   }
+  if (mode == PSE_DGRAD_ACT && mask) return PS_LAUNCHERS[16 + (p16 ? 2 : 0) + (w64 ? 1 : 0)](&p, lds, grid, (void*)st);
   return PS_LAUNCHERS[(p16 ? 8 : 0) + 2 * mode + (w64 ? 1 : 0)](&p, lds, grid, (void*)st);
 }
 #endif
@@ -718,6 +760,24 @@
 extern "C" int fdet_conv3x3_ps_dgrad_act(const void* dz_ps, const void* wpk, const void* act_ps, void* dx_ps, int N,
                                          int Cin, int Cout, int H, int W, float slope, void* stream) {
   return run_ps(PSE_DGRAD_ACT, dz_ps, wpk, nullptr, act_ps, dx_ps, PsPoolIO{}, N, Cout, Cin, H, W, slope, (hipStream_t)stream);
+}
+
+extern "C" size_t fdet_ps_mask_bytes(int N, int H, int W) {
+  PsGeo g;
+  PsStrips sp;
+  if (!ps_geo_strips(N, 64, H, W, g, sp)) return 0;
+  return (size_t)g.N * g.HP * g.WP * 8;
+}
+
+extern "C" int fdet_conv3x3_ps_fwd_m(const void* x_ps, const void* wpk, const float* bias, void* y_ps, void* mask, int N,
+                                     int Cin, int Cout, int H, int W, float slope, void* stream) {
+  return run_ps(PSE_FWD_FULL, x_ps, wpk, bias, nullptr, y_ps, PsPoolIO{}, N, Cin, Cout, H, W, slope, (hipStream_t)stream, false, mask);
+}
+
+extern "C" int fdet_conv3x3_ps_dgrad_act_m(const void* dz_ps, const void* wpk, const void* act_ps, const void* mask, void* dx_ps,
+                                           int N, int Cin, int Cout, int H, int W, float slope, void* stream) {
+  return run_ps(PSE_DGRAD_ACT, dz_ps, wpk, nullptr, act_ps, dx_ps, PsPoolIO{}, N, Cout, Cin, H, W, slope, (hipStream_t)stream, false,
+                const_cast<void*>(mask));
 }
 
 extern "C" int fdet_conv3x3_ps_fwd_pool(const void* x_ps, const void* wpk, const float* bias, const void* skip_ps,
@@ -744,6 +804,15 @@
                                              int Cin, int Cout, int H, int W, float slope, void* stream) {
   return run_ps(PSE_DGRAD_ACT, dz_ps, wpk, nullptr, act_ps, dx_ps, PsPoolIO{}, N, Cout, Cin, H, W, slope, (hipStream_t)stream, true);
 }
+extern "C" int fdet_conv3x3_ps_fwd_m_p16(const void* x_ps, const void* wpk, const float* bias, void* y_ps, void* mask, int N,
+                                         int Cin, int Cout, int H, int W, float slope, void* stream) {
+  return run_ps(PSE_FWD_FULL, x_ps, wpk, bias, nullptr, y_ps, PsPoolIO{}, N, Cin, Cout, H, W, slope, (hipStream_t)stream, true, mask);
+}
+extern "C" int fdet_conv3x3_ps_dgrad_act_m_p16(const void* dz_ps, const void* wpk, const void* act_ps, const void* mask,
+                                               void* dx_ps, int N, int Cin, int Cout, int H, int W, float slope, void* stream) {
+  return run_ps(PSE_DGRAD_ACT, dz_ps, wpk, nullptr, act_ps, dx_ps, PsPoolIO{}, N, Cout, Cin, H, W, slope, (hipStream_t)stream, true,
+                const_cast<void*>(mask));
+}
 extern "C" int fdet_conv3x3_ps_fwd_pool_p16(const void* x_ps, const void* wpk, const float* bias, const void* skip_ps,
                                             const float* drop_scale, void* pool_ps, float* pool_f32, unsigned char* route8,
                                             int N, int Cin, int Cout, int H, int W, float slope, void* stream) {
diff --git a/pytorch-face-detection-from-scratch_amd/ps.py b/pytorch-face-detection-from-scratch_amd/ps.py
--- a/pytorch-face-detection-from-scratch_amd/ps.py
+++ b/pytorch-face-detection-from-scratch_amd/ps.py
@@ -56,6 +56,28 @@
         return y
 
 
+class PsMask:
+
+    def __init__(self, N: int, H: int, W: int, device):
+        nbytes = int(lib().fdet_ps_mask_bytes(N, H, W))
+        if nbytes == 0:
+            raise FdetError(f"PsMask: unsupported map ({N},64,{H},{W})")
+        self.shape = (N, 64, H, W)
+        self.buf = torch.zeros(nbytes // 4, dtype=torch.int32, device=device)
+
+    @property
+    def data(self) -> int:
+        return self.buf.data_ptr()
+
+
+def _mask_ptr(mask, shape, name):
+    if mask is None:
+        return None
+    if not isinstance(mask, PsMask) or mask.shape != tuple(shape):
+        raise ValueError(f"{name}: expected a PsMask of shape {tuple(shape)}, got {getattr(mask, 'shape', type(mask))}")
+    return mask.data
+
+
 def halo_exchange(t: PsTensor, zero_only: bool = False, p16: bool = False) -> None:
     if t.strips <= 1:
         return
@@ -77,23 +99,33 @@
     return getattr(lib(), name + "_p16" if p16 else name)
 
 
-def conv3x3_ps_fwd(x: PsTensor, wpk: torch.Tensor, bias: torch.Tensor, y: PsTensor, slope: float = 0.2, p16: bool = False) -> None:
+def conv3x3_ps_fwd(x: PsTensor, wpk: torch.Tensor, bias: torch.Tensor, y: PsTensor, slope: float = 0.2, p16: bool = False,
+                   mask: PsMask = None) -> None:
     N, cin, H, W = x.shape
     cout = int(bias.shape[0])
     _same(y, (N, cout, H, W), "conv3x3_ps_fwd: y")
     if wpk.numel() != cout * cin * 9:
         raise ValueError("conv3x3_ps_fwd: packed weight size does not match (Cout,Cin)")
+    if mask is not None:
+        check(_fn("fdet_conv3x3_ps_fwd_m", p16)(x.data, ptr(wpk), ptr(bias), y.data, _mask_ptr(mask, y.shape, "conv3x3_ps_fwd: mask"),
+                                                N, cin, cout, H, W, float(slope), stream()), "fdet_conv3x3_ps_fwd_m")
+        return
     check(_fn("fdet_conv3x3_ps_fwd", p16)(x.data, ptr(wpk), ptr(bias), y.data, N, cin, cout, H, W, float(slope), stream()),
           "fdet_conv3x3_ps_fwd")
 
 
-def conv3x3_ps_dgrad_act(dz: PsTensor, wpk_bwd: torch.Tensor, act: PsTensor, dx: PsTensor, slope: float = 0.2, p16: bool = False) -> None:
+def conv3x3_ps_dgrad_act(dz: PsTensor, wpk_bwd: torch.Tensor, act: PsTensor, dx: PsTensor, slope: float = 0.2, p16: bool = False,
+                         mask: PsMask = None) -> None:
     N, cout, H, W = dz.shape
     cin = dx.shape[1]
     _same(dx, (N, cin, H, W), "conv3x3_ps_dgrad_act: dx")
     _same(act, (N, cin, H, W), "conv3x3_ps_dgrad_act: act")
     if wpk_bwd.numel() != cout * cin * 9:
         raise ValueError("conv3x3_ps_dgrad_act: packed weight size does not match (Cout,Cin)")
+    if mask is not None:
+        check(_fn("fdet_conv3x3_ps_dgrad_act_m", p16)(dz.data, ptr(wpk_bwd), act.data, _mask_ptr(mask, act.shape, "conv3x3_ps_dgrad_act: mask"),
+                                                      dx.data, N, cin, cout, H, W, float(slope), stream()), "fdet_conv3x3_ps_dgrad_act_m")
+        return
     check(_fn("fdet_conv3x3_ps_dgrad_act", p16)(dz.data, ptr(wpk_bwd), act.data, dx.data, N, cin, cout, H, W, float(slope),
                                                 stream()), "fdet_conv3x3_ps_dgrad_act")
 
```
